# psweens/VAN-GAN

Measured on AMD Instinct MI355X. Metric: train Mvoxels/s (VanGan.train_step, 128^3 bf16), higher is better.
Workload: dtype bf16; 1 GPU; VanGan.train_step, 128x128x128 volumes, batch 1 per GPU (global 1), clDice on, disc noise+dropout on; parallelism=dp1

## Files before the change

include/vangan_hip.h:

```cpp
#ifndef VANGAN_HIP_H
#define VANGAN_HIP_H
#include <stdint.h>
#ifdef __cplusplus
extern "C" {
#endif

typedef void* vg_stream_t;

#define VG_OK 0
#define VG_EINVAL (-1)
#define VG_ELDS (-2)
#define VG_ELAUNCH (-3)

#define VG_ACT_NONE 0
#define VG_ACT_RELU 1
#define VG_ACT_LRELU 2

#define VG_PAD_ZERO 0
#define VG_PAD_REFLECT 1

#define VG_MAX_TAPS 64

#define VG_STRIPES 8

const char* vg_status_string(int code);
int vg_set_stamp_buffer(void* dev_u64);
int vg_version(void);
int vg_storage16(void);
int vg_abi_sizeof(int which);

struct vg_actnorm_bwd_desc_s;
typedef struct {
    const float* gamma; const float* beta;
    const float* mult;
    float* scale; float* shift;
    float* mean; float* rstd;
    int32_t c_off, c_tot;
} vg_fin_job;
typedef struct {
    uint32_t* ticket;
    float count;
    float eps;
    int32_t njobs;
    vg_fin_job job[2];
} vg_fin_desc;
typedef struct {
    const void* src0;
    const void* src1;
    int32_t c_src0, c_src1;
    int32_t src0_shift;
    int32_t src_f32;
    int32_t N, D, H, W;
    const float* in_scale;
    const float* in_shift;
    int32_t act;
    const void* noise;
    int32_t noise_pad;
    int32_t istr;
    int32_t pad_mode;
    int32_t ntaps;
    int8_t tap_d[VG_MAX_TAPS], tap_h[VG_MAX_TAPS], tap_w[VG_MAX_TAPS];
    int32_t OD, OH, OW;
    int32_t ostr, ooff_d, ooff_h, ooff_w;
    int32_t BD, BH, BW;
    int32_t Cout;
    const void* wpacked;
    int32_t CK;
    const float* bias;
    const void* res;
    const float* res_scale;
    const float* res_shift;
    int32_t tanh_out;
    void* out;
    int32_t out_f32;
    int32_t accumulate;
    float* out_sums;
    int32_t f32;
    int32_t nclass;
    int32_t cls_tap0[9];
    const void* cls_w[8];
    int32_t cls_ooff[8][3];
    int32_t cls_iters[8][3];
    int32_t wpack;
    int32_t wpack_wmin;
    const struct vg_actnorm_bwd_desc_s* bstat;
    void* scratch;
    int64_t scratch_bytes;
    int32_t wlayout;
    const vg_fin_desc* fin;
    int32_t res_c1;
    const void* wpacked_up;
} vg_conv_desc;
#define VG_SCRATCH_CTR_BYTES 16384

int vg_conv3d(const vg_conv_desc* d, vg_stream_t stream);

int vg_conv3d_lds_bytes(const vg_conv_desc* d);
int vg_conv3d_plan(const vg_conv_desc* d, int32_t* plan4);
int vg_conv3d_thin_np(const vg_conv_desc* d);
int vg_conv3d_variant(const vg_conv_desc* d, char* buf, int buflen);
int vg_set_tuning(const char* key, int value, int reset);

int vg_pack_up_weights(const float* w, int Cin, int Cout, int c_up, void* out, vg_stream_t stream);

int vg_pack_weights(const float* w, int T, int Cin, int Cout, const int32_t* tap_idx_dev, int ntaps,
                    int transpose, int CK, void* out, int out_f32, vg_stream_t stream);
typedef struct {
    const float* w; const int32_t* tap_idx; void* out;
    int32_t Cin, Cout, ntaps, transpose, CK, out_f32;
    int32_t blk0, nblk;
    int32_t bn;
    int32_t pad_;
} vg_pack_item;
int vg_pack_weights_multi(const vg_pack_item* items_dev, int n, int total_blocks, vg_stream_t stream);
int vg_conv3d_dma_bn(const vg_conv_desc* d);
int64_t vg_conv3d_scratch_bytes(const vg_conv_desc* d);
int vg_pack_weights_dma(const float* w, int T, int Cin, int Cout, const int32_t* tap_idx_dev, int ntaps, int transpose, int bn,
                        void* out, vg_stream_t stream);
int vg_packed_ktot(int ntaps, int C, int CK);
int vg_packed_rows(int N);

int vg_conv3d_wgrad(const vg_conv_desc* d, const void* dy, int dy_f32, const int32_t* tap_idx_host,
                    int T_total, float* dw, float* db, float* scratch, int64_t scratch_bytes, vg_stream_t stream);
int vg_conv3d_wgrad_variant(const vg_conv_desc* d, int dy_f32, const int32_t* tap_idx_host, int T_total,
                            int64_t scratch_bytes, char* buf, int buflen);

int vg_in_finalize(const float* sums0, int c0, float count0, const float* sums1, int c1, float count1,
                   const float* gamma, const float* beta, const float* mult, int N, float eps,
                   float* scale, float* shift, float* mean, float* rstd, vg_stream_t stream);

typedef struct vg_actnorm_bwd_desc_s {
    const void* g; int32_t g_padded;
    const void* x; int32_t x_f32;
    const void* x1; int32_t c_x0; int32_t x0_shift;
    int32_t N, D, H, W, C;
    const float* scale; const float* shift;
    const float* mult;
    int32_t act; int32_t norm;
    const float* gamma; const float* mean; const float* rstd;
    float* red;
    void* dx; int32_t dx_f32; int32_t accumulate;
    int32_t dx_cstride, dx_coff;
    int32_t f32;
    float* dgamma;
    float* dbeta;
    int32_t* ticket;
    int32_t alias_n0, alias_shift, pgrad_n, pad_;
} vg_actnorm_bwd_desc;
int vg_actnorm_bwd_stats(const vg_actnorm_bwd_desc* d, vg_stream_t stream);
int vg_actnorm_bwd_apply(const vg_actnorm_bwd_desc* d, vg_stream_t stream);
int vg_actnorm_bwd_apply2(const vg_actnorm_bwd_desc* d1, const vg_actnorm_bwd_desc* d2, vg_stream_t stream);
int vg_actnorm_bwd(const vg_actnorm_bwd_desc* d, vg_stream_t stream);
int vg_stem_short_fwd_workgroups(int N, int64_t S);
int vg_stem_short_fwd(const float* x, int N, int64_t S, int C, const float* w, const float* gamma, const float* beta, float eps, int round16,
                      float* scale, float* shift, double* part, int G, unsigned* ticket, vg_stream_t stream);
int vg_stem_short_bwd_workgroups(int N, int64_t S, int C);
int vg_stem_short_bwd(const void* g, int g_f32, const float* x, int N, int64_t S, int C, const float* w, const float* gamma, float eps,
                      int round16, float* dw, float* dgamma, float* dbeta, double* part, int G, unsigned* ticket, vg_stream_t stream);
int vg_in_param_grads(const float* red, int N, int C, float* dgamma, float* dbeta, vg_stream_t stream);

int vg_concat_bwd(const void* g, int N, int D, int H, int W, int Cu, int Cs, void* dlow, void* dskip,
                  int f32, int accumulate, vg_stream_t stream);

int vg_shortcut_dgrad_concat(const vg_conv_desc* d, void* dlow, void* dskip, int c_low, int accumulate, vg_stream_t stream);
int vg_shortcut_dgrad_concat_norm(const vg_conv_desc* d, const vg_actnorm_bwd_desc* b, void* dlow, void* dskip, int c_low,
                                  int accumulate, vg_stream_t stream);

int vg_affine_add(const void* a, const float* a_scale, const float* a_shift, int a_act, const void* b, const float* b_scale,
                  const float* b_shift, int N, int64_t S, int C, void* out, int f32, vg_stream_t stream);

int vg_bias_grad(const void* dy, int f32, int64_t rows, int C, float* db, vg_stream_t stream);

int vg_pack_cell_weights(const float* w, int C, void* out, vg_stream_t stream);
int vg_cells_fold(const void* cells, int N, int D, int H, int W, float* dx, vg_stream_t stream);

int vg_tanh_bwd(const float* dy, const float* y, float* dpre, int64_t n, vg_stream_t stream);

int vg_minmax(const float* x, int B, int64_t S, float* mm4, vg_stream_t stream);
int vg_minmax_apply(const float* x, const float* mm4, int B, int64_t S, float* y, vg_stream_t stream);
int vg_minmax_bwd(const float* x, const float* y, const float* gy, const float* mm4, int B, int64_t S,
                  float* tmp2, float* dx, vg_stream_t stream);
int vg_bce(const float* t, const float* p, int64_t n, float* acc, float gscale, float* gp, int accumulate,
           vg_stream_t stream);
int vg_mse(const float* a, const float* b, int64_t n, float* acc, float gscale, float* gb, int accumulate,
           vg_stream_t stream);
int vg_mse_const(const void* x, int x_f32, float target, int64_t n, float* acc, float gscale, float* gx,
                 int accumulate, vg_stream_t stream);
int vg_ssim_fwd(const float* t, const float* p, int B, int D, int H, int W, float* acc, float* part,
                vg_stream_t stream);
int vg_ssim_bwd(const float* t, const float* p, const float* part, int B, int D, int H, int W, float gscale,
                float* gp, int accumulate, vg_stream_t stream);

int vg_soft_skel_fwd(const float* img, int B, int D, int H, int W, int iters, float* imgs, float* skels, void* aux,
                     vg_stream_t stream);
int vg_soft_skel_bwd(const float* imgs, const float* skels, const float* gskel, int B, int D, int H, int W,
                     int iters, float* work, float* gimg, const void* aux, vg_stream_t stream);
int vg_cldice_coef(const float* sums7, float w, float alpha, float* coef6, vg_stream_t stream);
int vg_cldice_grads(const float* t, const float* skel_t, const float* coef6, int64_t n, float* gskel_p, float* gp,
                    int accumulate, vg_stream_t stream);
int vg_dot_sums(const float* a, const float* b, int64_t n, float* sums3, vg_stream_t stream);
int vg_axpby(const float* a, float alpha, const float* b, float beta, int64_t n, float* y, int accumulate,
             vg_stream_t stream);

int vg_dense_head_fwd(const float* x, const float* mask, const float* w, const float* b, int N, int n, float* z, vg_stream_t stream);
int vg_dense_head_bwd(const float* x, const float* mask, const float* w, const float* gz, int N, int n, float* dx, float* dw, float* db,
                      vg_stream_t stream);
int vg_wasserstein_terms(const float* z, int B, float inv, float* acc2, float* gz_d, float* gz_g, vg_stream_t stream);

int vg_overlap_add(const float* win, int kx, int ky, int kz, int px, int py, int pz, int x0, int y0, int z0,
                   int X, int Y, int Z, float* pred, float* cnt, vg_stream_t stream);
int vg_divide_crop(const float* pred, const float* cnt, int X, int Y, int Z, int sx, int sy, int sz, int ox, int oy,
                   int oz, float* out, vg_stream_t stream);

int vg_adam_clip(float* w, const float* g, float* m, float* v, const int64_t* seg_off_dev, int T,
                 int64_t total, float* norms, float lr_t, float beta1, float beta2, float eps,
                 float clipnorm, float grad_scale, vg_stream_t stream);

#define VG_SN_MAX_ITEMS 8
#define VG_SN_MAX_PROJ 4
#define VG_SN_MAX_COUT 512
#define VG_SN_SLAB 65536
#define VG_SN_STATE 8
#define VG_SN_STATE_CUM 4
typedef struct {
    float* w; float* u; float* state;
    int32_t K, Cout;
    int32_t blk0, nblk;
} vg_sn_item;
int vg_spectral_norm_blocks(int K, int Cout);
int64_t vg_spectral_norm_scratch_bytes(int total_blocks);
int vg_spectral_norm(const vg_sn_item* items_dev, int T, int total_blocks, int n_proj, float* scratch, int64_t scratch_bytes,
                     vg_stream_t stream);

int vg_attn_gate_fwd(const void* skip, const void* phi, const float* w_theta, const float* b_theta, const float* w_psi,
                     const float* b_psi, int N, int D, int H, int W, int Cs, int Ci, int f32, void* gated, float* h, float* sums,
                     vg_stream_t stream);
int vg_attn_gate_bwd(const void* dg, const void* skip, const float* h, const void* phi, const float* w_theta,
                     const float* b_theta, const float* w_psi, int N, int D, int H, int W, int Cs, int Ci, int f32, void* dskip,
                     int accumulate, void* dphi, float* dw_theta, float* db_theta, float* dw_psi, float* db_psi,
                     vg_stream_t stream);

int vg_randn_bf16_dev(void* out, int64_t n, const float* std_dev, uint64_t seed, const uint64_t* offset_dev, uint64_t offset_add,
                      vg_stream_t stream);
int vg_dropout_mask_dev(float* out, int64_t n, float rate, uint64_t seed, const uint64_t* offset_dev, uint64_t offset_add,
                        vg_stream_t stream);
int vg_adam_clip_dev(float* w, const float* g, float* m, float* v, const int64_t* seg_off_dev, int T, int64_t total, float* norms,
                     const float* lr_t_dev, float beta1, float beta2, float eps, float clipnorm, float grad_scale, vg_stream_t stream);

int vg_set_step_params(void* block, uint64_t offset, float std, float lr0, float lr1, float lr2, float lr3, vg_stream_t stream);

int vg_local_exchange(float* buf, float* scratch, int64_t n, int workgroups, int min_us, vg_stream_t stream);

int vg_randn_bf16(void* out, int64_t n, float std, uint64_t seed, uint64_t offset, vg_stream_t stream);
int vg_dropout_mask(float* out, int64_t n, float rate, uint64_t seed, uint64_t offset, vg_stream_t stream);

int vg_crop_augment(const float* vol, int X, int Y, int Z, int C, int x0, int y0, int z0, int px, int py, int pz,
                    int flip_lr, int flip_ud, int rot_k, float* out, vg_stream_t stream);
int vg_crop_max(const float* vol, int X, int Y, int Z, int C, int x0, int y0, int z0, int px, int py, int pz,
                float* out, vg_stream_t stream);

int vg_memset_zero(void* p, int64_t nbytes, vg_stream_t stream);
int vg_copy_bytes(void* dst, const void* src, int64_t nbytes, vg_stream_t stream);

int vg_f32_to_bf16(const float* x, void* y, int64_t n, vg_stream_t stream);
int vg_bf16_to_f32(const void* x, float* y, int64_t n, vg_stream_t stream);

#ifdef __cplusplus
}
#endif
#endif
```

van_gan_amd/_lib.py:

```python
from __future__ import annotations

import ctypes as C
import os

import torch

from . import build as _build

VG_MAX_TAPS = 64
SN_STATE, SN_STATE_CUM, SN_MAX_PROJ = 8, 4, 4
ACT_NONE, ACT_RELU, ACT_LRELU = 0, 1, 2
PAD_ZERO, PAD_REFLECT = 0, 1
SCRATCH_CTR_BYTES = 16384

c_void_p, c_int, c_float, c_i64, c_u64 = C.c_void_p, C.c_int32, C.c_float, C.c_int64, C.c_uint64


class ConvDesc(C.Structure):
    _fields_ = [
        ('src0', c_void_p), ('src1', c_void_p), ('c_src0', c_int), ('c_src1', c_int), ('src0_shift', c_int),
        ('src_f32', c_int), ('N', c_int), ('D', c_int), ('H', c_int), ('W', c_int),
        ('in_scale', c_void_p), ('in_shift', c_void_p), ('act', c_int), ('noise', c_void_p), ('noise_pad', c_int),
        ('istr', c_int), ('pad_mode', c_int), ('ntaps', c_int),
        ('tap_d', C.c_int8 * VG_MAX_TAPS), ('tap_h', C.c_int8 * VG_MAX_TAPS), ('tap_w', C.c_int8 * VG_MAX_TAPS),
        ('OD', c_int), ('OH', c_int), ('OW', c_int), ('ostr', c_int), ('ooff_d', c_int), ('ooff_h', c_int),
        ('ooff_w', c_int), ('BD', c_int), ('BH', c_int), ('BW', c_int), ('Cout', c_int),
        ('wpacked', c_void_p), ('CK', c_int), ('bias', c_void_p),
        ('res', c_void_p), ('res_scale', c_void_p), ('res_shift', c_void_p), ('tanh_out', c_int),
        ('out', c_void_p), ('out_f32', c_int), ('accumulate', c_int), ('out_sums', c_void_p), ('f32', c_int),
        ('nclass', c_int), ('cls_tap0', c_int * 9), ('cls_w', c_void_p * 8), ('cls_ooff', (c_int * 3) * 8),
        ('cls_iters', (c_int * 3) * 8), ('wpack', c_int), ('wpack_wmin', c_int), ('bstat', c_void_p),
        ('scratch', c_void_p), ('scratch_bytes', c_i64), ('wlayout', c_int), ('fin', c_void_p), ('res_c1', c_int), ('wpacked_up', c_void_p),
    ]


class FinJob(C.Structure):
    _fields_ = [('gamma', c_void_p), ('beta', c_void_p), ('mult', c_void_p), ('scale', c_void_p), ('shift', c_void_p),
                ('mean', c_void_p), ('rstd', c_void_p), ('c_off', c_int), ('c_tot', c_int)]


class FinDesc(C.Structure):
    _fields_ = [('ticket', c_void_p), ('count', c_float), ('eps', c_float), ('njobs', c_int), ('job', FinJob * 2)]


class PackItem(C.Structure):
    _fields_ = [('w', c_void_p), ('tap_idx', c_void_p), ('out', c_void_p), ('Cin', c_int), ('Cout', c_int), ('ntaps', c_int),
                ('transpose', c_int), ('CK', c_int), ('out_f32', c_int), ('blk0', c_int), ('nblk', c_int), ('bn', c_int), ('pad_', c_int)]


class SnItem(C.Structure):
    _fields_ = [('w', c_void_p), ('u', c_void_p), ('state', c_void_p), ('K', c_int), ('Cout', c_int), ('blk0', c_int), ('nblk', c_int)]


class ActNormBwdDesc(C.Structure):
    _fields_ = [
        ('g', c_void_p), ('g_padded', c_int), ('x', c_void_p), ('x_f32', c_int),
        ('x1', c_void_p), ('c_x0', c_int), ('x0_shift', c_int),
        ('N', c_int), ('D', c_int), ('H', c_int), ('W', c_int), ('C', c_int),
        ('scale', c_void_p), ('shift', c_void_p), ('mult', c_void_p), ('act', c_int), ('norm', c_int),
        ('gamma', c_void_p), ('mean', c_void_p), ('rstd', c_void_p), ('red', c_void_p),
        ('dx', c_void_p), ('dx_f32', c_int), ('accumulate', c_int), ('dx_cstride', c_int), ('dx_coff', c_int),
        ('f32', c_int), ('dgamma', c_void_p), ('dbeta', c_void_p), ('ticket', c_void_p),
        ('alias_n0', c_int), ('alias_shift', c_int), ('pgrad_n', c_int), ('pad_', c_int),
    ]


_SIGS = {
    'vg_version': ([], c_int),
    'vg_storage16': ([], c_int),
    'vg_abi_sizeof': ([c_int], c_int),
    'vg_set_stamp_buffer': ([c_void_p], c_int),
    'vg_conv3d': ([C.POINTER(ConvDesc), c_void_p], c_int),
    'vg_conv3d_lds_bytes': ([C.POINTER(ConvDesc)], c_int),
    'vg_conv3d_plan': ([C.POINTER(ConvDesc), C.POINTER(C.c_int32)], c_int),
    'vg_conv3d_variant': ([C.POINTER(ConvDesc), C.c_char_p, c_int], c_int),
    'vg_conv3d_thin_np': ([C.POINTER(ConvDesc)], c_int),
    'vg_set_tuning': ([C.c_char_p, c_int, c_int], c_int),
    'vg_conv3d_wgrad_variant': ([C.POINTER(ConvDesc), c_int, C.POINTER(c_int), c_int, c_i64, C.c_char_p, c_int], c_int),
    'vg_pack_weights': ([c_void_p, c_int, c_int, c_int, c_void_p, c_int, c_int, c_int, c_void_p, c_int, c_void_p], c_int),
    'vg_pack_weights_multi': ([c_void_p, c_int, c_int, c_void_p], c_int),
    'vg_crop_augment': ([c_void_p] + [c_int] * 13 + [c_void_p, c_void_p], c_int),
    'vg_crop_max': ([c_void_p] + [c_int] * 10 + [c_void_p, c_void_p], c_int),
    'vg_conv3d_dma_bn': ([C.POINTER(ConvDesc)], c_int),
    'vg_conv3d_scratch_bytes': ([C.POINTER(ConvDesc)], c_i64),
    'vg_pack_weights_dma': ([c_void_p, c_int, c_int, c_int, c_void_p, c_int, c_int, c_int, c_void_p, c_void_p], c_int),
    'vg_packed_ktot': ([c_int, c_int, c_int], c_int),
    'vg_packed_rows': ([c_int], c_int),
    'vg_conv3d_wgrad': ([C.POINTER(ConvDesc), c_void_p, c_int, C.POINTER(c_int), c_int, c_void_p, c_void_p, c_void_p, c_i64,
                         c_void_p], c_int),
    'vg_in_finalize': ([c_void_p, c_int, c_float, c_void_p, c_int, c_float, c_void_p, c_void_p, c_void_p, c_int,
                        c_float, c_void_p, c_void_p, c_void_p, c_void_p, c_void_p], c_int),
    'vg_actnorm_bwd_stats': ([C.POINTER(ActNormBwdDesc), c_void_p], c_int),
    'vg_actnorm_bwd_apply': ([C.POINTER(ActNormBwdDesc), c_void_p], c_int),
    'vg_actnorm_bwd_apply2': ([C.POINTER(ActNormBwdDesc), C.POINTER(ActNormBwdDesc), c_void_p], c_int),
    'vg_actnorm_bwd': ([C.POINTER(ActNormBwdDesc), c_void_p], c_int),
    'vg_stem_short_fwd_workgroups': ([c_int, c_i64], c_int),
    'vg_stem_short_fwd': ([c_void_p, c_int, c_i64, c_int, c_void_p, c_void_p, c_void_p, C.c_float, c_int, c_void_p, c_void_p, c_void_p, c_int, c_void_p,
                          c_void_p], c_int),
    'vg_stem_short_bwd_workgroups': ([c_int, c_i64, c_int], c_int),
    'vg_stem_short_bwd': ([c_void_p, c_int, c_void_p, c_int, c_i64, c_int, c_void_p, c_void_p, C.c_float, c_int, c_void_p, c_void_p, c_void_p,
                          c_void_p, c_int, c_void_p, c_void_p], c_int),
    'vg_in_param_grads': ([c_void_p, c_int, c_int, c_void_p, c_void_p, c_void_p], c_int),
    'vg_concat_bwd': ([c_void_p, c_int, c_int, c_int, c_int, c_int, c_int, c_void_p, c_void_p, c_int, c_int, c_void_p], c_int),
    'vg_shortcut_dgrad_concat': ([C.POINTER(ConvDesc), c_void_p, c_void_p, c_int, c_int, c_void_p], c_int),
    'vg_shortcut_dgrad_concat_norm': ([C.POINTER(ConvDesc), C.POINTER(ActNormBwdDesc), c_void_p, c_void_p, c_int, c_int, c_void_p], c_int),
    'vg_affine_add': ([c_void_p, c_void_p, c_void_p, c_int, c_void_p, c_void_p, c_void_p, c_int, c_i64, c_int, c_void_p, c_int, c_void_p], c_int),
    'vg_bias_grad': ([c_void_p, c_int, c_i64, c_int, c_void_p, c_void_p], c_int),
    'vg_pack_cell_weights': ([c_void_p, c_int, c_void_p, c_void_p], c_int),
    'vg_cells_fold': ([c_void_p, c_int, c_int, c_int, c_int, c_void_p, c_void_p], c_int),
    'vg_tanh_bwd': ([c_void_p, c_void_p, c_void_p, c_i64, c_void_p], c_int),
    'vg_minmax': ([c_void_p, c_int, c_i64, c_void_p, c_void_p], c_int),
    'vg_minmax_apply': ([c_void_p, c_void_p, c_int, c_i64, c_void_p, c_void_p], c_int),
    'vg_minmax_bwd': ([c_void_p, c_void_p, c_void_p, c_void_p, c_int, c_i64, c_void_p, c_void_p, c_void_p], c_int),
    'vg_bce': ([c_void_p, c_void_p, c_i64, c_void_p, c_float, c_void_p, c_int, c_void_p], c_int),
    'vg_mse': ([c_void_p, c_void_p, c_i64, c_void_p, c_float, c_void_p, c_int, c_void_p], c_int),
    'vg_mse_const': ([c_void_p, c_int, c_float, c_i64, c_void_p, c_float, c_void_p, c_int, c_void_p], c_int),
    'vg_ssim_fwd': ([c_void_p, c_void_p, c_int, c_int, c_int, c_int, c_void_p, c_void_p, c_void_p], c_int),
    'vg_ssim_bwd': ([c_void_p, c_void_p, c_void_p, c_int, c_int, c_int, c_int, c_float, c_void_p, c_int, c_void_p], c_int),
    'vg_soft_skel_fwd': ([c_void_p, c_int, c_int, c_int, c_int, c_int, c_void_p, c_void_p, c_void_p, c_void_p], c_int),
    'vg_soft_skel_bwd': ([c_void_p, c_void_p, c_void_p, c_int, c_int, c_int, c_int, c_int, c_void_p, c_void_p, c_void_p, c_void_p], c_int),
    'vg_cldice_coef': ([c_void_p, c_float, c_float, c_void_p, c_void_p], c_int),
    'vg_cldice_grads': ([c_void_p, c_void_p, c_void_p, c_i64, c_void_p, c_void_p, c_int, c_void_p], c_int),
    'vg_dense_head_fwd': ([c_void_p, c_void_p, c_void_p, c_void_p, c_int, c_int, c_void_p, c_void_p], c_int),
    'vg_dense_head_bwd': ([c_void_p, c_void_p, c_void_p, c_void_p, c_int, c_int, c_void_p, c_void_p, c_void_p, c_void_p], c_int),
    'vg_wasserstein_terms': ([c_void_p, c_int, c_float, c_void_p, c_void_p, c_void_p, c_void_p], c_int),
    'vg_dot_sums': ([c_void_p, c_void_p, c_i64, c_void_p, c_void_p], c_int),
    'vg_overlap_add': ([c_void_p] + [c_int] * 12 + [c_void_p, c_void_p, c_void_p], c_int),
    'vg_divide_crop': ([c_void_p, c_void_p] + [c_int] * 9 + [c_void_p, c_void_p], c_int),
    'vg_axpby': ([c_void_p, c_float, c_void_p, c_float, c_i64, c_void_p, c_int, c_void_p], c_int),
    'vg_adam_clip': ([c_void_p, c_void_p, c_void_p, c_void_p, c_void_p, c_int, c_i64, c_void_p, c_float, c_float,
                      c_float, c_float, c_float, c_float, c_void_p], c_int),
    'vg_spectral_norm_blocks': ([c_int, c_int], c_int),
    'vg_spectral_norm_scratch_bytes': ([c_int], c_i64),
    'vg_spectral_norm': ([c_void_p, c_int, c_int, c_int, c_void_p, c_i64, c_void_p], c_int),
    'vg_attn_gate_fwd': ([c_void_p] * 6 + [c_int] * 7 + [c_void_p] * 4, c_int),
    'vg_attn_gate_bwd': ([c_void_p] * 7 + [c_int] * 7 + [c_void_p, c_int] + [c_void_p] * 6, c_int),
    'vg_local_exchange': ([c_void_p, c_void_p, c_i64, c_int, c_int, c_void_p], c_int),
    'vg_randn_bf16': ([c_void_p, c_i64, c_float, c_u64, c_u64, c_void_p], c_int),
    'vg_dropout_mask': ([c_void_p, c_i64, c_float, c_u64, c_u64, c_void_p], c_int),
    'vg_randn_bf16_dev': ([c_void_p, c_i64, c_void_p, c_u64, c_void_p, c_u64, c_void_p], c_int),
    'vg_dropout_mask_dev': ([c_void_p, c_i64, c_float, c_u64, c_void_p, c_u64, c_void_p], c_int),
    'vg_adam_clip_dev': ([c_void_p, c_void_p, c_void_p, c_void_p, c_void_p, c_int, c_i64, c_void_p, c_void_p, c_float,
                          c_float, c_float, c_float, c_float, c_void_p], c_int),
    'vg_set_step_params': ([c_void_p, c_u64, c_float, c_float, c_float, c_float, c_float, c_void_p], c_int),
    'vg_pack_up_weights': ([c_void_p, c_int, c_int, c_int, c_void_p, c_void_p], c_int),
    'vg_memset_zero': ([c_void_p, c_i64, c_void_p], c_int),
    'vg_copy_bytes': ([c_void_p, c_void_p, c_i64, c_void_p], c_int),
    'vg_f32_to_bf16': ([c_void_p, c_void_p, c_i64, c_void_p], c_int),
    'vg_bf16_to_f32': ([c_void_p, c_void_p, c_i64, c_void_p], c_int),
}

EXPORTS = sorted(list(_SIGS.keys()) + ['vg_status_string'])


def _load(path=None, storage16=0):
    path = _build.LIB if path is None else path
    if not os.path.exists(path) or (_build.needs_build() and os.environ.get('VG_NO_REBUILD') != '1'):
        _build.build()
    lib = C.CDLL(path)
    for name, (args, ret) in _SIGS.items():
        fn = getattr(lib, name)
        fn.argtypes = args
        fn.restype = ret
    lib.vg_status_string.argtypes = [c_int]
    lib.vg_status_string.restype = C.c_char_p
    for which, mirror in ((0, ConvDesc), (1, ActNormBwdDesc), (2, PackItem), (3, FinDesc), (4, SnItem)):
        got = lib.vg_abi_sizeof(which)
        if got != C.sizeof(mirror):
            raise ImportError('libvangan_hip.so ABI mismatch: sizeof(%s) is %d in the library, %d in van_gan_amd/_lib.py '
                              '(stale build? remove %s and rebuild)' % (mirror.__name__, got, C.sizeof(mirror), path))
    if lib.vg_storage16() != storage16:
        raise ImportError('%s stores %s in its 16-bit buffers, expected %s' % (path, ('bf16', 'fp16')[lib.vg_storage16()], ('bf16', 'fp16')[storage16]))
    return lib


lib = _load()
_lib_h = None


def lib_fp16():
    global _lib_h
    if _lib_h is None:
        _lib_h = _load(_build.LIB_H, 1)
    return _lib_h


class VgError(RuntimeError):
    pass


def check(rc: int, what: str = '') -> int:
    if rc < 0:
        raise VgError('%s failed: %s (%d)' % (what or 'libvangan_hip call', lib.vg_status_string(rc).decode(), rc))
    return rc
```

van_gan_amd/csrc/vg_pointwise.hip:

```cpp
#include "vg_common.h"
#include "vg_c1k3.h"
#include <stdlib.h>

namespace {

struct PW {
    const void* x; int x_f32;
    const float* scale; const float* shift; int act;
    const void* w; int kc_pad, CK;
    const float* bias;
    void* out; int out_f32, accumulate, tanh_out;
    float* sums;
    const void* dy; int dy_f32;
    float* dw; float* db;
    int N, C; int64_t S;
    VgFin fin;
};

__device__ __forceinline__ float pw_slope(int act) { return act == VG_ACT_RELU ? 0.f : (act == VG_ACT_LRELU ? VG_LRELU : 1.f); }
__device__ __forceinline__ float ld_single(const void* p, int f32, int64_t i) {
    return f32 ? ld_global((const float*)p + i) : ld_global((const bf16_t*)p + i);
}

template <typename T, int G>
// ... 27 lines not shown
                float x[8]; raw_unpack(r[k][g], x);
#pragma unroll
                for (int j = 0; j < 8; ++j) {
                    float y = x[j] * sc[g * 8 + j] + sf[g * 8 + j];
                    y = fmaxf(y, y * slope);
                    a += rnd<T>(y) * wv[g * 8 + j];
                }
            }
            const size_t o = (size_t)n * p.S + v + k * stride;
            if (p.tanh_out && !p.accumulate) a = tanhf(a);
            if (p.out_f32) { float* q = (float*)p.out + o; a = p.accumulate ? *q + a : a; *q = a; }
            else { bf16_t* q = (bf16_t*)p.out + o; const bf16_t h = f2bf(p.accumulate ? bf2f(*q) + a : a); *q = h; a = bf2f(h); }
            s1 += a; s2 += a * a;
        }
    }
    if (p.sums) {
        __shared__ float red[8];
#pragma unroll
        for (int o = 32; o > 0; o >>= 1) { s1 += __shfl_xor(s1, o); s2 += __shfl_xor(s2, o); }
        if ((threadIdx.x & 63) == 0) { red[(threadIdx.x >> 6) * 2] = s1; red[(threadIdx.x >> 6) * 2 + 1] = s2; }
        __syncthreads();
        if (threadIdx.x < 2) {
            const int stripe = blockIdx.x & (VG_STRIPES - 1);
            atomicAdd(&p.sums[((size_t)stripe * gridDim.y + n) * 2 + threadIdx.x],
                      red[threadIdx.x] + red[2 + threadIdx.x] + red[4 + threadIdx.x] + red[6 + threadIdx.x]);
        }
    }
}

template <typename T>
__global__ __launch_bounds__(256) void pw_1toc_kernel(const PW p) {
    __shared__ float part[16 * 256];
    const int n = blockIdx.y, tid = threadIdx.x;
    const int gpc = p.C >> 3, vpb = 256 / gpc;
    const int cg = tid % gpc, vl = tid / gpc;
    const bool live = tid < gpc * vpb;
    float wv[8], bv[8], s1[8], s2[8];
#pragma unroll
    for (int j = 0; j < 8; ++j) {
        wv[j] = live ? ld1<T>((const T*)p.w + (size_t)(cg * 8 + j) * p.kc_pad) : 0.f;
        bv[j] = (live && p.bias) ? p.bias[cg * 8 + j] : 0.f;
        s1[j] = 0.f; s2[j] = 0.f;
    }
    const float sc = p.scale ? p.scale[n] : 1.f, sf = p.scale ? p.shift[n] : 0.f, slope = pw_slope(p.act);
    const int64_t xoff = (int64_t)n * p.S;
    T* ob = (T*)p.out + (size_t)n * p.S * p.C + cg * 8;
    const int64_t stride = (int64_t)gridDim.x * vpb;
    if (live)
    for (int64_t v = (int64_t)blockIdx.x * vpb + vl; v < p.S; v += 4 * stride) {
        float xs[4]; Raw8<T> old[4];
#pragma unroll
        for (int k = 0; k < 4; ++k) {
            const int64_t vv = v + k * stride < p.S ? v + k * stride : v;
            xs[k] = ld_single(p.x, p.x_f32, xoff + vv);
            if (p.accumulate) raw_load(old[k], ob + vv * p.C);
        }
#pragma unroll
        for (int k = 0; k < 4; ++k) {
            if (v + k * stride >= p.S) continue;
            float y = xs[k] * sc + sf;
            y = rnd<T>(fmaxf(y, y * slope));
            float o[8];
#pragma unroll
            for (int j = 0; j < 8; ++j) o[j] = y * wv[j] + bv[j];
            if (p.accumulate) {
                float q[8]; raw_unpack(old[k], q);
#pragma unroll
                for (int j = 0; j < 8; ++j) o[j] += q[j];
            }
            store8<T>(ob + (v + k * stride) * p.C, o);
#pragma unroll
            for (int j = 0; j < 8; ++j) { const float r = rnd<T>(o[j]); s1[j] += r; s2[j] += r * r; }
        }
    }
    if (!p.sums) return;
#pragma unroll
    for (int j = 0; j < 8; ++j) { part[(2 * j) * 256 + tid] = live ? s1[j] : 0.f; part[(2 * j + 1) * 256 + tid] = live ? s2[j] : 0.f; }
    __syncthreads();
    const int stripe = blockIdx.x & (VG_STRIPES - 1);
    float* dst = p.sums + ((size_t)stripe * gridDim.y + n) * p.C * 2;
    for (int o = tid; o < p.C * 2; o += 256) {
        const int ch = o >> 1, mom = o & 1, g8 = ch >> 3, j = ch & 7;
        const float* src = part + (2 * j + mom) * 256 + g8;
        float a = 0.f;
        for (int t = 0; t < vpb; ++t) a += src[t * gpc];
        atomicAdd(&dst[o], a);
    }
    if (p.fin.ticket) vg_fin_tail(p.fin, p.sums, gridDim.y, p.C, gridDim.x * gridDim.y, (int*)part);
}

template <typename T, int GI>
__global__ __launch_bounds__(256) void pw_ctoc_kernel(const PW p, int Cin, int Ktot) {
    const int n = blockIdx.y, tid = threadIdx.x;
    const int gpc = p.C >> 3, vpb = 256 / gpc;
    const int cg = tid % gpc, vl = tid / gpc;
    if (tid >= gpc * vpb) return;
    float wv[GI * 8][8], bv[8];
#pragma unroll
    for (int k = 0; k < GI * 8; ++k)
#pragma unroll
        for (int j = 0; j < 8; ++j)
            wv[k][j] = ld1<T>((const T*)p.w + (size_t)(cg * 8 + j) * Ktot + (k / p.CK) * p.kc_pad + (k % p.CK));
#pragma unroll
    for (int j = 0; j < 8; ++j) bv[j] = p.bias ? p.bias[cg * 8 + j] : 0.f;
    const T* xb = (const T*)p.x + (size_t)n * p.S * Cin;
    T* ob = (T*)p.out + (size_t)n * p.S * p.C + cg * 8;
    const int64_t stride = (int64_t)gridDim.x * vpb;
    for (int64_t v = (int64_t)blockIdx.x * vpb + vl; v < p.S; v += 2 * stride) {
        Raw8<T> xr[2][GI], old[2];
#pragma unroll
        for (int k = 0; k < 2; ++k) {
            const int64_t vv = v + k * stride < p.S ? v + k * stride : v;
#pragma unroll
            for (int g = 0; g < GI; ++g) raw_load(xr[k][g], xb + vv * Cin + g * 8);
            if (p.accumulate) raw_load(old[k], ob + vv * p.C);
        }
#pragma unroll
        for (int k = 0; k < 2; ++k) {
            if (v + k * stride >= p.S) continue;
            float o[8];
#pragma unroll
            for (int j = 0; j < 8; ++j) o[j] = bv[j];
#pragma unroll
            for (int g = 0; g < GI; ++g) {
                float x[8]; raw_unpack(xr[k][g], x);
#pragma unroll
                for (int e = 0; e < 8; ++e)
#pragma unroll
                    for (int j = 0; j < 8; ++j) o[j] += x[e] * wv[g * 8 + e][j];
            }
            if (p.accumulate) {
                float q[8]; raw_unpack(old[k], q);
#pragma unroll
                for (int j = 0; j < 8; ++j) o[j] += q[j];
            }
            store8<T>(ob + (v + k * stride) * p.C, o);
        }
    }
}

struct PWG {
    const bf16_t* x0; const bf16_t* x1; int c0, c1, Cin, sh;
    const bf16_t* w; int Ktot, CK, kc_pad;
    const float* bias; bf16_t* out; float* sums;
    int N, ID, IH, IW, OD, OH, OW, istr;
    int BD, BH, BW, ostr, od0, oh0, ow0;
    int Cout; int SO;
    unsigned long long* stamps;
    bf16_t* dlow; bf16_t* dskip; int sc0, sacc;
    const bf16_t* ng; const bf16_t* nx0; const bf16_t* nx1;
    const float* n_scale; const float* n_shift; const float* n_mean; const float* n_rstd; const float* n_gamma; const float* n_mult;
    VgFin fin;
    const float* n_red; float* n_dgamma; float* n_dbeta; int n_act;
};
}
extern unsigned long long* g_vg_stamps;
namespace {
typedef __attribute__((ext_vector_type(2))) float pw_f32x2;
typedef __attribute__((ext_vector_type(2))) unsigned pw_u32x2;
typedef __attribute__((ext_vector_type(4))) unsigned pw_u32x4;

__device__ __forceinline__ void vg_reflect_fold8(const bf16_t* gp, int C, int D, int H, int W, int dk, int hk, int wk, float* g) {
    const int PH = H + 2, PW_ = W + 2;
    const int md = dk == 1 ? 0 : (dk == D - 2 ? D + 1 : -1), mh = hk == 1 ? 0 : (hk == H - 2 ? H + 1 : -1), mw = wk == 1 ? 0 : (wk == W - 2 ? W + 1 : -1);
    Raw8<bf16_t> rr[7];
    bool val[7];
#pragma unroll
    for (int t = 1; t < 8; ++t) {
        const int qd = (t & 4) ? md : dk + 1, qh = (t & 2) ? mh : hk + 1, qw = (t & 1) ? mw : wk + 1;
        val[t - 1] = (qd | qh | qw) >= 0;
        raw_load(rr[t - 1], gp + (val[t - 1] ? ((size_t)(qd * PH + qh) * PW_ + qw) * C : ((size_t)((dk + 1) * PH + hk + 1) * PW_ + wk + 1) * C));
    }
#pragma unroll
    for (int t = 0; t < 7; ++t) {
        float r[8]; raw_unpack(rr[t], r);
#pragma unroll
        for (int j = 0; j < 8; ++j) g[j] += val[t] ? r[j] : 0.f;
    }
}

template <int KS, int NB, bool GEO, bool ACC, bool STATS, int SPLIT = 0>
__global__ __launch_bounds__(256) void pw_gemm_kernel(const PWG p) {
    static_assert(!SPLIT || (ACC && !GEO && !STATS), "SPLIT: accumulating, same-grid launches");
    constexpr int MS = (KS * NB <= 2) ? 4 : 2;
    __shared__ float stat[NB * 32];
    const int tid = threadIdx.x, lane = tid & 63, wave = tid >> 6, r = lane & 15, kg = lane >> 4;
    const int n = blockIdx.y;
    if (p.stamps && lane == 0) p.stamps[((size_t)blockIdx.x * 4 + wave) * 8] = __builtin_amdgcn_s_memrealtime();
    float* ntab = nullptr;
    if constexpr (SPLIT == 2) {
        __shared__ float ntab_s[5 * NB * 16];
        ntab = ntab_s;
        constexpr int C = NB * 16;
        if (tid < C && tid < p.Cout) {
            const int nc = n * p.Cout + tid;
            const size_t total = (size_t)p.N * p.Cout * 2;
            float r0 = 0.f, r1 = 0.f;
#pragma unroll
            for (int t = 0; t < VG_STRIPES; ++t) { r0 += p.n_red[t * total + (size_t)nc * 2]; r1 += p.n_red[t * total + (size_t)nc * 2 + 1]; }
            if (p.n_dgamma && blockIdx.x == 0) { atomicAdd(&p.n_dbeta[tid], r0); atomicAdd(&p.n_dgamma[tid], r1); }
            const float cnt = (float)p.SO, rs = p.n_rstd[nc], mu = p.n_mean[nc], gr = p.n_gamma[tid] * rs;
            const float k1 = gr * r0 / cnt, k2 = gr * r1 / cnt, cc = k2 * rs;
            ntab_s[tid] = p.n_scale ? p.n_scale[nc] : 1.f;
            ntab_s[C + tid] = p.n_scale ? p.n_shift[nc] : 0.f;
            ntab_s[2 * C + tid] = gr * (p.n_mult ? p.n_mult[nc] : 1.f);
            ntab_s[3 * C + tid] = k1 - cc * mu;
            ntab_s[4 * C + tid] = cc;
        }
        __syncthreads();
    }
    bf16x8 wA[NB][KS];
    pw_f32x2 e_b[NB][2];
#pragma unroll
    for (int nb = 0; nb < NB; ++nb) {
        const int co = nb * 16 + r;
#pragma unroll
        for (int ks = 0; ks < KS; ++ks) {
            const int c = ks * 32 + kg * 8;
            wA[nb][ks] = (bf16x8){0, 0, 0, 0, 0, 0, 0, 0};
            if (co < p.Cout && c < p.Cin) wA[nb][ks] = *(const bf16x8*)(p.w + (size_t)co * p.Ktot + (c / p.CK) * p.kc_pad + (c % p.CK));
        }
#pragma unroll
        for (int i = 0; i < 4; ++i) {
            const int cb = nb * 16 + kg * 4 + i;
            e_b[nb][i >> 1][i & 1] = (p.bias && cb < p.Cout) ? p.bias[cb] : 0.f;
        }
    }
    if (p.stamps) { asm volatile("s_waitcnt vmcnt(0)" ::: "memory"); if (lane == 0) p.stamps[((size_t)blockIdx.x * 4 + wave) * 8 + 1] = __builtin_amdgcn_s_memrealtime(); }
    float s1[NB][4], s2[NB][4];
#pragma unroll
    for (int nb = 0; nb < NB; ++nb)
#pragma unroll
        for (int i = 0; i < 4; ++i) { s1[nb][i] = 0.f; s2[nb][i] = 0.f; }
    if (STATS) { if (tid < NB * 32) stat[tid] = 0.f; __syncthreads(); }
    const int OHW = p.OH * p.OW;
    const int ID2 = p.ID >> p.sh, IH2 = p.IH >> p.sh, IW2 = p.IW >> p.sh;
    const int nwt = (p.SO + MS * 16 - 1) / (MS * 16);
    const int jodd = kg & 1, chof = (kg & ~1) * 4;
    auto split_store = [&](int wt, int jp, int nb, float* o, bool ok, size_t vox) {
        if (nb * 16 < p.sc0) {
#pragma unroll
            for (int i = 0; i < 8; ++i) { o[i] += __shfl_xor(o[i], 1); o[i] += __shfl_xor(o[i], 2); o[i] += __shfl_xor(o[i], 4); }
            if (ok && (r & 7) == 0) {
                const size_t cidx = (size_t)n * (p.SO >> 3) + (size_t)wt * (MS * 2) + (jp + jodd) * 2 + (r >> 3);
                bf16_t* dst = p.dlow + cidx * p.sc0 + nb * 16 + chof;
                if (p.sacc & 1) { float old[8]; load8<bf16_t>(dst, old); for (int i = 0; i < 8; ++i) o[i] += old[i]; }
                store8<bf16_t>(dst, o);
            }
        } else if (ok) {
            bf16_t* dst = p.dskip + vox * (p.Cout - p.sc0) + (nb * 16 - p.sc0) + chof;
            if (p.sacc & 2) { float old[8]; load8<bf16_t>(dst, old); for (int i = 0; i < 8; ++i) o[i] += old[i]; }
            store8<bf16_t>(dst, o);
        }
    };
    for (int wt = blockIdx.x * 4 + wave; wt < nwt; wt += gridDim.x * 4) {
        bf16x8 xb[MS][KS];
        bool vok[MS], oks[MS / 2];
        size_t i0s[MS], i1s[MS], ovs[MS / 2];
        size_t ovf[MS / 2];
        int fdhw[MS / 2];
#pragma unroll
        for (int jp = 0; jp < MS; jp += 2) {
            size_t ovp[2];
#pragma unroll
            for (int e = 0; e < 2; ++e) {
                const int i = jp + e;
                const int v = wt * (MS * 16) + i * 16 + r;
                vok[i] = v < p.SO;
                const int vc = vok[i] ? v : p.SO - 1;
                if (GEO) {
                    const int od = vc / OHW, rem = vc - od * OHW, oh = rem / p.OW, ow = rem - oh * p.OW;
                    const int id = od * p.istr, ih = oh * p.istr, iw = ow * p.istr;
                    i0s[i] = (((size_t)n * ID2 + (id >> p.sh)) * IH2 + (ih >> p.sh)) * IW2 + (iw >> p.sh);
                    i1s[i] = (((size_t)n * p.ID + id) * p.IH + ih) * p.IW + iw;
                    ovp[e] = (((size_t)n * p.BD + od * p.ostr + p.od0) * p.BH + oh * p.ostr + p.oh0) * p.BW + ow * p.ostr + p.ow0;
                } else if (SPLIT) {
                    const int cb = vc >> 3, j = vc & 7;
                    const int CW = p.OW >> 1, CHW = (p.OH >> 1) * CW;
                    const int cd = cb / CHW, rem = cb - cd * CHW, ch = rem / CW, cw = rem - ch * CW;
                    const int fd = 2 * cd + (j >> 2), fh = 2 * ch + ((j >> 1) & 1), fw = 2 * cw + (j & 1);
                    const int vf = (fd * p.OH + fh) * p.OW + fw;
                    i0s[i] = i1s[i] = ovp[e] = (size_t)n * p.SO + vf;
                    if (e == jodd) fdhw[jp >> 1] = fd | (fh << 10) | (fw << 20);
                } else {
                    i0s[i] = i1s[i] = ovp[e] = (size_t)n * p.SO + vc;
                }
            }
            ovf[jp >> 1] = jodd ? ovp[1] : ovp[0];
            ovs[jp >> 1] = (jodd ? ovp[1] : ovp[0]) * p.Cout + chof;
            oks[jp >> 1] = jodd ? vok[jp + 1] : vok[jp];
        }
        Raw8<bf16_t> oldv[ACC ? MS / 2 : 1][ACC ? NB : 1];
        if (ACC && SPLIT != 2) {
#pragma unroll
            for (int jh = 0; jh < MS / 2; ++jh)
#pragma unroll
                for (int nb = 0; nb < NB; ++nb) raw_load(oldv[jh][nb], p.out + ovs[jh] + (nb * 16 < p.Cout ? nb * 16 : 0));
            if (p.stamps) { asm volatile("s_waitcnt vmcnt(0)" ::: "memory"); if (lane == 0) p.stamps[((size_t)blockIdx.x * 4 + wave) * 8 + 3] = __builtin_amdgcn_s_memrealtime(); }
        }
#pragma unroll
        for (int i = 0; i < MS; ++i)
#pragma unroll
            for (int ks = 0; ks < KS; ++ks) {
                const int c = ks * 32 + kg * 8;
                const bool cok = c < p.Cin;
                const int ce = cok ? c : c % p.Cin;
                const bf16_t* q = ce < p.c0 ? p.x0 + i0s[i] * p.c0 + ce : p.x1 + i1s[i] * p.c1 + (ce - p.c0);
                Raw8<bf16_t> t;
                raw_load(t, q);
                raw_mask(t, cok);
                xb[i][ks] = t.v;
            }
        if (p.stamps) { asm volatile("s_waitcnt vmcnt(0)" ::: "memory"); if (lane == 0) p.stamps[((size_t)blockIdx.x * 4 + wave) * 8 + 2] = __builtin_amdgcn_s_memrealtime(); }
        if constexpr (SPLIT == 2) {
            const int PH = p.OH + 2, PW_ = p.OW + 2;
            size_t gi[MS / 2], li[MS / 2], si[MS / 2];
            bool bord[MS / 2];
#pragma unroll
            for (int jh = 0; jh < MS / 2; ++jh) {
                const int fd = fdhw[jh] & 1023, fh = (fdhw[jh] >> 10) & 1023, fw = fdhw[jh] >> 20;
                gi[jh] = ((((size_t)n * (p.OD + 2) + fd + 1) * PH + fh + 1) * PW_ + fw + 1) * p.Cout + chof;
                li[jh] = ((((size_t)n * (p.OD >> 1) + (fd >> 1)) * (p.OH >> 1) + (fh >> 1)) * (p.OW >> 1) + (fw >> 1)) * p.sc0 + chof;
                si[jh] = ovf[jh] * (p.Cout - p.sc0) + chof;
                bord[jh] = fd == 1 || fd == p.OD - 2 || fh == 1 || fh == p.OH - 2 || fw == 1 || fw == p.OW - 2;
            }
            constexpr int C = NB * 16;
            const float slope = pw_slope(p.n_act);
            Raw8<bf16_t> gq[NB][MS / 2], xq[NB][MS / 2];
#pragma unroll
            for (int nb = 0; nb < NB; ++nb)
#pragma unroll
                for (int jh = 0; jh < MS / 2; ++jh) {
                    raw_load(gq[nb][jh], p.ng + gi[jh] + nb * 16);
                    raw_load(xq[nb][jh], nb * 16 < p.sc0 ? p.nx0 + li[jh] + nb * 16 : p.nx1 + si[jh] + (nb * 16 - p.sc0));
                }
#pragma unroll
            for (int nb = 0; nb < NB; ++nb) {
                f32x4 a[MS];
#pragma unroll
                for (int i = 0; i < MS; ++i) {
                    a[i] = (f32x4){0.f, 0.f, 0.f, 0.f};
#pragma unroll
                    for (int ks = 0; ks < KS; ++ks) a[i] = VG_MFMA16(wA[nb][ks], xb[i][ks], a[i]);
                }
                const float* tb = ntab + nb * 16 + chof;
#pragma unroll
                for (int jp = 0; jp < MS; jp += 2) {
                    float o[8];
#pragma unroll
                    for (int i = 0; i < 4; ++i) {
                        const pw_u32x2 x = __builtin_amdgcn_permlane16_swap(__float_as_uint(a[jp][i]), __float_as_uint(a[jp + 1][i]), false, false);
                        o[i] = __uint_as_float(x[0]); o[4 + i] = __uint_as_float(x[1]);
                    }
                    float q[8], xv[8];
                    raw_unpack(gq[nb][jp >> 1], q); raw_unpack(xq[nb][jp >> 1], xv);
                    if (bord[jp >> 1]) {
                        const int fd = fdhw[jp >> 1] & 1023, fh = (fdhw[jp >> 1] >> 10) & 1023, fw = fdhw[jp >> 1] >> 20;
                        vg_reflect_fold8(p.ng + (size_t)n * (p.OD + 2) * PH * PW_ * p.Cout + nb * 16 + chof, p.Cout, p.OD, p.OH, p.OW, fd, fh, fw, q);
                    }
#pragma unroll
                    for (int i = 0; i < 8; ++i) {
                        const float pre = xv[i] * tb[i] + tb[C + i];
                        const float m = (pre > 0.f || p.n_act == VG_ACT_NONE) ? 1.f : slope;
                        o[i] += tb[2 * C + i] * m * q[i] - tb[3 * C + i] - tb[4 * C + i] * xv[i];
                    }
                    split_store(wt, jp, nb, o, oks[jp >> 1], ovf[jp >> 1]);
                }
                __builtin_amdgcn_sched_barrier(0);
            }
            continue;
        }
        f32x4 acc[MS][NB];
#pragma unroll
        for (int i = 0; i < MS; ++i)
#pragma unroll
            for (int nb = 0; nb < NB; ++nb) {
                acc[i][nb] = (f32x4){0.f, 0.f, 0.f, 0.f};
#pragma unroll
                for (int ks = 0; ks < KS; ++ks) acc[i][nb] = VG_MFMA16(wA[nb][ks], xb[i][ks], acc[i][nb]);
            }
#pragma unroll
        for (int jp = 0; jp < MS; jp += 2) {
            const bool ok = oks[jp >> 1];
            const size_t ob = ovs[jp >> 1];
#pragma unroll
            for (int nb = 0; nb < NB; ++nb) {
                if (nb * 16 >= p.Cout) continue;
                bf16_t* optr = p.out + ob + nb * 16;
                pw_u32x4 outv;
                if (ACC) {
                    float o[8];
#pragma unroll
                    for (int i = 0; i < 4; ++i) {
                        const pw_u32x2 x = __builtin_amdgcn_permlane16_swap(__float_as_uint(acc[jp][nb][i] + e_b[nb][i >> 1][i & 1]),
                                                                            __float_as_uint(acc[jp + 1][nb][i] + e_b[nb][i >> 1][i & 1]), false, false);
                        o[i] = __uint_as_float(x[0]); o[4 + i] = __uint_as_float(x[1]);
                    }
                    float q[8]; raw_unpack(oldv[ACC ? jp >> 1 : 0][ACC ? nb : 0], q);
                    if (SPLIT) {
#pragma unroll
                        for (int i = 0; i < 8; ++i) o[i] += q[i];
                        split_store(wt, jp, nb, o, ok, ovf[jp >> 1]);
                        continue;
                    }
                    bf16x8 pk;
#pragma unroll
                    for (int i = 0; i < 8; ++i) pk[i] = (short)f2bf(o[i] + q[i]);
                    outv = __builtin_bit_cast(pw_u32x4, pk);
                } else {
                    bf16x4 pk[2];
#pragma unroll
                    for (int e = 0; e < 2; ++e) {
                        pw_f32x2 v0 = {acc[jp + e][nb][0], acc[jp + e][nb][1]}, v1 = {acc[jp + e][nb][2], acc[jp + e][nb][3]};
                        v0 += e_b[nb][0]; v1 += e_b[nb][1];
                        pk[e] = (bf16x4){(short)f2bf(v0[0]), (short)f2bf(v0[1]), (short)f2bf(v1[0]), (short)f2bf(v1[1])};
                        if (STATS) {
                            const bool okv = vok[jp + e];
#pragma unroll
                            for (int i = 0; i < 4; ++i) {
                                const float qv = okv ? bf2f((bf16_t)pk[e][i]) : 0.f;
                                s1[nb][i] += qv; s2[nb][i] += qv * qv;
                            }
                        }
                    }
                    const pw_u32x2 wa = __builtin_bit_cast(pw_u32x2, pk[0]), wb = __builtin_bit_cast(pw_u32x2, pk[1]);
                    const pw_u32x2 x0 = __builtin_amdgcn_permlane16_swap(wa[0], wb[0], false, false);
                    const pw_u32x2 x1 = __builtin_amdgcn_permlane16_swap(wa[1], wb[1], false, false);
                    outv = (pw_u32x4){x0[0], x1[0], x0[1], x1[1]};
                }
                if (ok) *(pw_u32x4*)optr = outv;
            }
        }
    }
    if (p.stamps && lane == 0) { asm volatile("s_waitcnt vmcnt(0)" ::: "memory"); p.stamps[((size_t)blockIdx.x * 4 + wave) * 8 + 7] = __builtin_amdgcn_s_memrealtime(); }
    if (STATS && p.sums) {
#pragma unroll
        for (int nb = 0; nb < NB; ++nb)
#pragma unroll
            for (int i = 0; i < 4; ++i) {
                float a = s1[nb][i], b = s2[nb][i];
#pragma unroll
                for (int o = 1; o < 16; o <<= 1) { a += __shfl_xor(a, o); b += __shfl_xor(b, o); }
                if (r == 0) { atomicAdd(&stat[(nb * 16 + 4 * kg + i) * 2], a); atomicAdd(&stat[(nb * 16 + 4 * kg + i) * 2 + 1], b); }
            }
        __syncthreads();
        if (tid < NB * 32) {
            const int co = tid >> 1;
            const int stripe = blockIdx.x & (VG_STRIPES - 1);
            if (co < p.Cout) atomicAdd(&p.sums[(((size_t)stripe * gridDim.y + n) * p.Cout + co) * 2 + (tid & 1)], stat[tid]);
        }
        if (p.fin.ticket) vg_fin_tail(p.fin, p.sums, gridDim.y, p.Cout, gridDim.x * gridDim.y, (int*)stat);
    }
}

struct PWW {
    const bf16_t* x0; const bf16_t* x1; int c0, c1, Cin, sh;
    const bf16_t* dy; int Cout;
    int N, ID, IH, IW, OD, OH, OW, istr, SO;
    int gin, roles, rp, vpb;
    float* dw; float* db; float* part; int dw_elems;
};

__global__ __launch_bounds__(256) void pw_wgrad_cc_kernel(const PWW p) {
    __shared__ float red[4 * 64 * 16];
    const int tid = threadIdx.x, n = blockIdx.y;
    const int role = tid & (p.rp - 1), vl = tid / p.rp;
    const bool live = role < p.roles;
    const int rl = live ? role : 0;
    const int cg = rl % p.gin, cob = rl / p.gin, c = cg * 8;
    const bool from0 = c < p.c0;
    const float bmask = cg == 0 ? 1.f : 0.f;
    pw_f32x2 acc[8][8], bs[8];
#pragma unroll
    for (int i = 0; i < 8; ++i) {
        bs[i] = (pw_f32x2){0.f, 0.f};
#pragma unroll
        for (int j = 0; j < 8; ++j) acc[i][j] = (pw_f32x2){0.f, 0.f};
    }
    const int ID2 = p.ID >> p.sh, IH2 = p.IH >> p.sh, IW2 = p.IW >> p.sh;
    const int step = gridDim.x * p.vpb;
    int v = blockIdx.x * p.vpb + vl;
    const int OHW = p.OH * p.OW;
    int od = v / OHW, oh = (v - od * OHW) / p.OW, ow = v - od * OHW - oh * p.OW;
    const int sd = step / OHW, sh_ = (step - sd * OHW) / p.OW, sw = step - sd * OHW - sh_ * p.OW;
    const bf16_t* xb = from0 ? p.x0 + c : p.x1 + (c - p.c0);
    const int cs = from0 ? p.c0 : p.c1, shx = from0 ? p.sh : 0;
    const int XD = from0 ? ID2 : p.ID, XH = from0 ? IH2 : p.IH, XW = from0 ? IW2 : p.IW;
    const bf16_t* yb = p.dy + (size_t)n * p.SO * p.Cout + cob * 16;
// ... 224 lines not shown
        atomicAdd(&dst[o], a);
    }
    if (p.fin.ticket) vg_fin_tail(p.fin, p.sums, gridDim.y, p.C, gridDim.x * gridDim.y, (int*)part);
}

template <typename T, typename S>
__global__ __launch_bounds__(256) void c1k3_wgrad_kernel(C1K3 p) {
    __shared__ float part[20 * 256];
    const int n = blockIdx.y, tid = threadIdx.x;
    const int gpc = p.C >> 3, roles = 3 * gpc, qpb = 256 / roles;
    const int role = tid % roles, cg = role % gpc, a = role / gpc, ql = tid / roles;
    const bool live = tid < roles * qpb;
    if (p.scale) { p.sc = p.scale[n]; p.sf = p.shift[n]; }
    float acc[80];
#pragma unroll
    for (int i = 0; i < 80; ++i) acc[i] = 0.f;
    const int64_t nq = (int64_t)p.D * p.H * p.W4;
    if (live)
    for (int64_t q = (int64_t)blockIdx.x * qpb + ql; q < nq; q += (int64_t)gridDim.x * qpb) {
        const int wq = (int)(q % p.W4); const int64_t r = q / p.W4;
        const int h = (int)(r % p.H), d = (int)(r / p.H), w0 = wq * 4;
        float xv[1][3][6];
        c1_window<T, S, 1>(p, n, d, h, w0, a, xv);
        const T* yb = (const T*)p.dy + (((size_t)n * p.D + d) * p.H + h) * p.W * p.C + cg * 8;
        Raw8<T> yr[4];
#pragma unroll
        for (int v = 0; v < 4; ++v) raw_load(yr[v], yb + (size_t)min(w0 + v, p.W - 1) * p.C);
#pragma unroll
        for (int v = 0; v < 4; ++v) {
            float g[8]; raw_unpack(yr[v], g);
            const bool okv = w0 + v < p.W;
#pragma unroll
            for (int c = 0; c < 8; ++c) g[c] = okv ? g[c] : 0.f;
#pragma unroll
            for (int b = 0; b < 3; ++b)
#pragma unroll
                for (int j = 0; j < 3; ++j) {
                    const float x = xv[0][b][v + j];
#pragma unroll
                    for (int c = 0; c < 8; ++c) acc[(b * 3 + j) * 8 + c] += x * g[c];
                }
            if (a == 0) {
#pragma unroll
                for (int c = 0; c < 8; ++c) acc[72 + c] += g[c];
            }
        }
    }
#pragma unroll
    for (int chunk = 0; chunk < 4; ++chunk) {
        __syncthreads();
#pragma unroll
        for (int i = 0; i < 20; ++i) part[i * 256 + tid] = live ? acc[chunk * 20 + i] : 0.f;
        __syncthreads();
        for (int o = tid; o < roles * 20; o += 256) {
            const int i = o / roles, ro = o - i * roles;
            const float* src = part + i * 256 + ro;
            float sacc = 0.f;
            for (int t = 0; t < qpb; ++t) sacc += src[t * roles];
            const int val = chunk * 20 + i, rcg = ro % gpc, ra = ro / gpc;
            if (val < 72) {
                const int b = val / 24, j = (val / 8) % 3, c = val & 7;
                atomicAdd(&p.dw[(size_t)(((ra * 3 + b) * 3) + j) * p.C + rcg * 8 + c], sacc);
            } else if (ra == 0 && p.db) atomicAdd(&p.db[rcg * 8 + (val - 72)], sacc);
        }
    }
}

bool c1k3_fill(const vg_conv_desc* d, C1K3& p) {
    if (d->c_src0 != 1 || d->src1 || d->c_src1 || d->wpack != 3 || d->ntaps != 9 || d->istr != 1 || d->noise || d->nclass > 1) return false;
    if (d->Cout < 8 || d->Cout > 32 || (d->Cout % 8)) return false;
    if (d->OD != d->D || d->OH != d->H || d->OW != d->W) return false;
    for (int t = 0; t < 9; ++t)
        if (d->tap_d[t] != d->tap_d[0] + t / 3 || d->tap_h[t] != d->tap_h[0] + t % 3 || d->tap_w[t] != 0) return false;
    p.x = d->src0; p.x_f32 = d->src_f32; p.sc = 1.f; p.sf = 0.f; p.scale = d->in_scale; p.shift = d->in_shift; p.act = d->act;
    p.pad_mode = d->pad_mode; p.D = d->D; p.H = d->H; p.W = d->W; p.C = d->Cout; p.W4 = (d->W + 3) / 4;
    p.td0 = d->tap_d[0]; p.th0 = d->tap_h[0]; p.tw0 = d->wpack_wmin;
    p.CK = d->CK; p.Ktot = ((9 * d->CK + 31) / 32) * 32;
    return true;
}

bool pw_enabled() { return vg_tune("PW", 1) != 0; }
bool pw_shape_ok(const vg_conv_desc* d) {
    if (!pw_enabled() || d->ntaps != 1 || d->tap_d[0] || d->tap_h[0] || d->tap_w[0]) return false;
    if (d->istr != 1 || d->src1 || d->c_src1 || d->src0_shift || d->noise || d->wpack || d->nclass > 1) return false;
    if (d->OD != d->D || d->OH != d->H || d->OW != d->W) return false;
    return true;
}
int pw_blocks(int64_t work_items, int N) {
    int64_t b = (work_items + 255) / 256;
    const int64_t cap = 2047 / (N > 0 ? N : 1);
    if (b > cap) b = cap;
    return b < 1 ? 1 : (int)b;
}

template <bool GEO, bool ACC, bool STATS>
bool pwg_launch(int KS, int NB, dim3 grid, hipStream_t s, const PWG& p) {
#define PWG_CASE(ks, nb) if (KS == ks && NB == nb) { hipLaunchKernelGGL((pw_gemm_kernel<ks, nb, GEO, ACC, STATS>), grid, dim3(256), 0, s, p); return true; }
    PWG_CASE(1, 1) PWG_CASE(1, 2) PWG_CASE(1, 3) PWG_CASE(1, 4) PWG_CASE(1, 6) PWG_CASE(2, 1) PWG_CASE(2, 2) PWG_CASE(3, 2)
    PWG_CASE(4, 4) PWG_CASE(6, 4) PWG_CASE(2, 8)
#undef PWG_CASE
    return false;
}
template <int SPLIT>
bool pwg_launch_split(int KS, int NB, dim3 grid, hipStream_t s, const PWG& p) {
#define PWG_CASE(ks, nb) if (KS == ks && NB == nb) { hipLaunchKernelGGL((pw_gemm_kernel<ks, nb, false, true, false, SPLIT>), grid, dim3(256), 0, s, p); return true; }
    PWG_CASE(1, 3) PWG_CASE(1, 6) PWG_CASE(2, 6)
#undef PWG_CASE
    return false;
}
bool pwg_case_ok(int KS, int NB) {
    static const int tab[][2] = {{1, 1}, {1, 2}, {1, 3}, {1, 4}, {1, 6}, {2, 1}, {2, 2}, {3, 2}, {4, 4}, {6, 4}, {2, 8}};
    for (auto& t : tab) if (t[0] == KS && t[1] == NB) return true;
    return false;
}
int pw_gemm_conv(const vg_conv_desc* d, hipStream_t s) {
    if (!pw_enabled() || !vg_tune("PW_GEMM", 1)) return 1;
    if (d->ntaps != 1 || d->tap_d[0] || d->tap_h[0] || d->tap_w[0] || d->noise || d->wpack || d->nclass > 1) return 1;
    if (d->f32 || d->src_f32 || d->out_f32 || d->in_scale || d->act != VG_ACT_NONE || d->res || d->tanh_out) return 1;
    const int Cin = d->c_src0 + d->c_src1;
    if (Cin < 8 || (Cin % 8) || (d->c_src1 && (d->c_src0 % 8)) || d->Cout < 16 || (d->Cout % 16) || (d->CK % 8)) return 1;
    if (d->c_src1 && !d->src1) return 1;
    if (d->src0_shift && ((d->D | d->H | d->W) & 1)) return 1;
    if (d->istr < 1 || d->ostr < 1 || (d->OD - 1) * d->istr >= d->D || (d->OH - 1) * d->istr >= d->H || (d->OW - 1) * d->istr >= d->W) return 1;
    if (d->accumulate && d->out_sums) return 1;
    const int64_t SO = (int64_t)d->OD * d->OH * d->OW;
    if (SO < 1 || SO > (1 << 30)) return 1;
    const int KS = (Cin + 31) / 32, NB = d->Cout / 16;
    if (!pwg_case_ok(KS, NB)) return 1;
    const bool geo = d->src0_shift || d->istr != 1 || d->ostr != 1 || d->ooff_d || d->ooff_h || d->ooff_w || d->BD != d->OD || d->BH != d->OH
                     || d->BW != d->OW || d->OD != d->D || d->OH != d->H || d->OW != d->W;
    PWG p = {};
    p.x0 = (const bf16_t*)d->src0; p.x1 = (const bf16_t*)(d->c_src1 ? d->src1 : d->src0); p.c0 = d->c_src0; p.c1 = d->c_src1 ? d->c_src1 : 1;
    p.Cin = Cin; p.sh = d->src0_shift ? 1 : 0;
    p.w = (const bf16_t*)d->wpacked; p.CK = d->CK; p.kc_pad = ((d->CK + 31) / 32) * 32; p.Ktot = ((Cin + d->CK - 1) / d->CK) * p.kc_pad;
    p.bias = d->bias; p.out = (bf16_t*)d->out; p.sums = d->out_sums;
    p.N = d->N; p.ID = d->D; p.IH = d->H; p.IW = d->W; p.OD = d->OD; p.OH = d->OH; p.OW = d->OW; p.istr = d->istr;
    p.BD = d->BD; p.BH = d->BH; p.BW = d->BW; p.ostr = d->ostr; p.od0 = d->ooff_d; p.oh0 = d->ooff_h; p.ow0 = d->ooff_w;
    p.Cout = d->Cout; p.SO = (int)SO; p.stamps = g_vg_stamps;
    p.fin = vg_fin_of(d);
    const int MS = (KS * NB <= 2) ? 4 : 2;
    const int64_t nwt = (SO + MS * 16 - 1) / (MS * 16);
    int64_t b = (nwt + 3) / 4;
    const int capt = vg_tune("PW_GEMM_CAP", 2047);
    const int64_t cap = (capt / d->N) > 0 ? (capt / d->N) : 1;
    if (b > cap) b = cap;
    const dim3 grid((int)b, d->N);
    if (vg_dry("pw_gemm<%d,%d,g%d,a%d>", KS, NB, (geo || !d->accumulate) ? 1 : 0, d->accumulate ? 1 : 0)) return VG_OK;
    bool ok;
    if (!d->accumulate) { ok = pwg_launch<true, false, true>(KS, NB, grid, s, p); if (ok && p.sums && p.fin.ticket) vg_fin_done = true; }
    else ok = geo ? pwg_launch<true, true, false>(KS, NB, grid, s, p) : pwg_launch<false, true, false>(KS, NB, grid, s, p);
    return ok ? vg_check_launch() : 1;
}

int pw_gemm_split(const vg_conv_desc* d, const vg_actnorm_bwd_desc* nb_, void* dlow, void* dskip, int c_low, int acc, hipStream_t s) {
    if (!pw_enabled() || !vg_tune("PW_GEMM", 1) || !vg_tune("PW_SPLIT", 1)) return 1;
    if (d->ntaps != 1 || d->tap_d[0] || d->tap_h[0] || d->tap_w[0] || d->noise || d->wpack || d->nclass > 1) return 1;
    if (d->f32 || d->src_f32 || d->out_f32 || d->in_scale || d->act != VG_ACT_NONE || d->res || d->tanh_out || d->out_sums || d->bias) return 1;
    const int Cin = d->c_src0;
    if (d->c_src1 || d->src0_shift || Cin < 8 || (Cin % 8) || d->Cout < 32 || (d->Cout % 16) || (d->CK % 8) || (!d->accumulate && !nb_)) return 1;
    if (nb_) {
        if (!nb_->norm || !nb_->g_padded || nb_->f32 || nb_->x_f32 || !nb_->g || !nb_->x || !nb_->x1 || !nb_->x0_shift || nb_->c_x0 != c_low) return 1;
        if (nb_->C != d->Cout || nb_->N != d->N || nb_->D != d->D || nb_->H != d->H || nb_->W != d->W || !nb_->gamma || !nb_->mean || !nb_->rstd || !nb_->red) return 1;
        if (d->D < 4 || d->H < 4 || d->W < 4 || d->D > 1023 || d->H > 1023 || d->W > 1023) return 1;
    }
    if (c_low < 16 || (c_low % 16) || c_low >= d->Cout) return 1;
    if (d->istr != 1 || d->ostr != 1 || d->ooff_d || d->ooff_h || d->ooff_w || d->BD != d->OD || d->BH != d->OH || d->BW != d->OW
        || d->OD != d->D || d->OH != d->H || d->OW != d->W || ((d->D | d->H | d->W) & 1)) return 1;
    const int64_t SO = (int64_t)d->OD * d->OH * d->OW;
    if (SO < 8 || SO > (1 << 30)) return 1;
    const int KS = (Cin + 31) / 32, NB = d->Cout / 16;
    if (!((KS == 1 && (NB == 3 || NB == 6)) || (KS == 2 && NB == 6))) return 1;
    PWG p = {};
    p.x0 = (const bf16_t*)d->src0; p.x1 = p.x0; p.c0 = Cin; p.c1 = 1; p.Cin = Cin; p.sh = 0;
    p.w = (const bf16_t*)d->wpacked; p.CK = d->CK; p.kc_pad = ((d->CK + 31) / 32) * 32; p.Ktot = ((Cin + d->CK - 1) / d->CK) * p.kc_pad;
    p.bias = nullptr; p.out = (bf16_t*)d->out; p.sums = nullptr;
    p.N = d->N; p.ID = d->D; p.IH = d->H; p.IW = d->W; p.OD = d->OD; p.OH = d->OH; p.OW = d->OW; p.istr = 1;
    p.BD = d->BD; p.BH = d->BH; p.BW = d->BW; p.ostr = 1;
    p.Cout = d->Cout; p.SO = (int)SO; p.stamps = g_vg_stamps;
    p.dlow = (bf16_t*)dlow; p.dskip = (bf16_t*)dskip; p.sc0 = c_low; p.sacc = acc;
    if (nb_) {
        p.ng = (const bf16_t*)nb_->g; p.nx0 = (const bf16_t*)nb_->x; p.nx1 = (const bf16_t*)nb_->x1;
        p.n_scale = nb_->scale; p.n_shift = nb_->shift; p.n_mean = nb_->mean; p.n_rstd = nb_->rstd; p.n_gamma = nb_->gamma; p.n_mult = nb_->mult;
        p.n_red = nb_->red; p.n_dgamma = (nb_->dgamma && nb_->dbeta) ? nb_->dgamma : nullptr; p.n_dbeta = nb_->dbeta; p.n_act = nb_->act;
    }
    const int MS = (KS * NB <= 2) ? 4 : 2;
    const int64_t nwt = (SO + MS * 16 - 1) / (MS * 16);
    int64_t b = (nwt + 3) / 4;
    const int capt = vg_tune("PW_GEMM_CAP", 2047);
    const int64_t cap = (capt / d->N) > 0 ? (capt / d->N) : 1;
    if (b > cap) b = cap;
    if (vg_dry("pw_gemm_split<%d,%d,n%d>", KS, NB, nb_ ? 1 : 0)) return VG_OK;
    const bool ok = nb_ ? pwg_launch_split<2>(KS, NB, dim3((int)b, d->N), s, p) : pwg_launch_split<1>(KS, NB, dim3((int)b, d->N), s, p);
    return ok ? vg_check_launch() : 1;
}

int pw_wgrad_cc(const vg_conv_desc* d, const void* dy, int dy_f32, int T_total, float* dw, float* db, float* scratch,
                int64_t scratch_bytes, hipStream_t s) {
    if (!pw_enabled() || !vg_tune("PW_WGRAD_CC", 1)) return 1;
    if (T_total != 1 || d->ntaps != 1 || d->tap_d[0] || d->tap_h[0] || d->tap_w[0] || d->noise || d->wpack || d->nclass > 1) return 1;
    if (d->f32 || d->src_f32 || dy_f32 || d->in_scale || d->act != VG_ACT_NONE) return 1;
    const int Cin = d->c_src0 + d->c_src1;
    if (Cin < 8 || (Cin % 8) || (d->c_src1 && (d->c_src0 % 8)) || d->Cout < 16 || (d->Cout % 16)) return 1;
    if (d->c_src1 && !d->src1) return 1;
    if (d->src0_shift && ((d->D | d->H | d->W) & 1)) return 1;
    if (d->istr < 1 || (d->OD - 1) * d->istr >= d->D || (d->OH - 1) * d->istr >= d->H || (d->OW - 1) * d->istr >= d->W) return 1;
    const int64_t SO = (int64_t)d->OD * d->OH * d->OW;
    if (SO < 1 || SO > (1 << 30)) return 1;
    PWW p = {};
    p.gin = Cin / 8; p.roles = p.gin * (d->Cout / 16);
    if (p.roles > vg_tune("PW_WGRAD_ROLES", 16)) return 1;
    p.rp = pow2_ceil(p.roles); p.vpb = 256 / p.rp;
    p.x0 = (const bf16_t*)d->src0; p.x1 = (const bf16_t*)(d->c_src1 ? d->src1 : d->src0); p.c0 = d->c_src0; p.c1 = d->c_src1 ? d->c_src1 : 1;
    p.Cin = Cin; p.sh = d->src0_shift ? 1 : 0; p.dy = (const bf16_t*)dy; p.Cout = d->Cout;
    p.N = d->N; p.ID = d->D; p.IH = d->H; p.IW = d->W; p.OD = d->OD; p.OH = d->OH; p.OW = d->OW; p.istr = d->istr; p.SO = (int)SO;
    p.dw = dw; p.db = db; p.dw_elems = Cin * d->Cout;
    int64_t b = (SO + (int64_t)p.vpb * 8 - 1) / ((int64_t)p.vpb * 8);
    const int capt = vg_tune("PW_WGRAD_CAP", 511);
    const int64_t cap = (capt / d->N) > 0 ? (capt / d->N) : 1;
    if (b > cap) b = cap;
    if (b < 1) b = 1;
    const int nslab = (int)b * d->N;
    p.part = (nslab > 4 && scratch && (int64_t)nslab * p.dw_elems * 4 <= scratch_bytes) ? scratch : nullptr;
    if (vg_dry("pw_wgrad_cc<r%d>|part%d", p.roles, p.part ? 1 : 0)) return VG_OK;
    hipLaunchKernelGGL(pw_wgrad_cc_kernel, dim3((int)b, d->N), dim3(256), 0, s, p);
    if (p.part) vg_launch_reduce_partials(p.part, nslab, p.dw_elems, dw, s);
    return vg_check_launch();
}

}

extern "C" int vg_shortcut_dgrad_concat(const vg_conv_desc* d, void* dlow, void* dskip, int c_low, int accumulate, vg_stream_t stream) {
    vg_begin();
    if (!d || !d->src0 || !d->out || !d->wpacked || !dlow || !dskip) return VG_EINVAL;
    return pw_gemm_split(d, nullptr, dlow, dskip, c_low, accumulate, (hipStream_t)stream);
}
extern "C" int vg_shortcut_dgrad_concat_norm(const vg_conv_desc* d, const vg_actnorm_bwd_desc* b, void* dlow, void* dskip, int c_low,
                                             int accumulate, vg_stream_t stream) {
    vg_begin();
    if (!d || !b || !d->src0 || !d->wpacked || !dlow || !dskip) return VG_EINVAL;
    if (!vg_tune("PW_SPLIT_NORM", 1)) return 1;
    return pw_gemm_split(d, b, dlow, dskip, c_low, accumulate, (hipStream_t)stream);
}

int vg_pointwise_conv(const vg_conv_desc* d, hipStream_t s) {
    if (pw_enabled() && !d->res && !d->tanh_out && !d->accumulate && d->ostr == 1 && !d->ooff_d && !d->ooff_h && !d->ooff_w
        && d->BD == d->OD && d->BH == d->OH && d->BW == d->OW && !(d->out_f32 && !d->f32)) {
        { const int mrc = c1m_fwd(d, s); if (mrc <= 0) return mrc; }
        C1K3 c;
        if (c1k3_fill(d, c)) {
            c.w = d->wpacked; c.bias = d->bias; c.out = d->out; c.sums = d->out_sums;
            c.fin = vg_fin_of(d);
            const int qpb = 256 / (c.C >> 3);
            int64_t b = ((int64_t)c.D * c.H * c.W4 + qpb - 1) / qpb;
            const int64_t cap = (2047 / d->N) > 0 ? (2047 / d->N) : 1;
            if (b > cap) b = cap;
            const dim3 grid((int)b, d->N);
            if (vg_dry("c1k3_fwd<%s,%s>", d->f32 ? "f32" : "bf16", d->src_f32 ? "f32" : "bf16")) return VG_OK;
            if (d->f32) {
                if (d->src_f32) hipLaunchKernelGGL((c1k3_fwd_kernel<float, float>), grid, dim3(256), 0, s, c);
                else hipLaunchKernelGGL((c1k3_fwd_kernel<float, bf16_t>), grid, dim3(256), 0, s, c);
            } else {
                if (d->src_f32) hipLaunchKernelGGL((c1k3_fwd_kernel<bf16_t, float>), grid, dim3(256), 0, s, c);
                else hipLaunchKernelGGL((c1k3_fwd_kernel<bf16_t, bf16_t>), grid, dim3(256), 0, s, c);
            }
            if (c.sums && c.fin.ticket) vg_fin_done = true;
            return vg_check_launch();
        }
    }
    { const int grc = pw_gemm_conv(d, s); if (grc <= 0) return grc; }
    if (!pw_shape_ok(d) || d->res) return 1;
    if (d->ostr != 1 || d->ooff_d || d->ooff_h || d->ooff_w || d->BD != d->OD || d->BH != d->OH || d->BW != d->OW) return 1;
    if (d->tanh_out && d->accumulate) return 1;
    const int Cin = d->c_src0;
    PW p = {};
    p.x = d->src0; p.x_f32 = d->src_f32; p.scale = d->in_scale; p.shift = d->in_shift; p.act = d->act;
    p.w = d->wpacked; p.CK = d->CK; p.kc_pad = ((d->CK + 31) / 32) * 32;
    p.bias = d->bias; p.out = d->out; p.out_f32 = (d->out_f32 || d->f32) ? 1 : 0; p.accumulate = d->accumulate; p.tanh_out = d->tanh_out;
    p.sums = d->out_sums; p.N = d->N; p.S = (int64_t)d->D * d->H * d->W;
    if (d->Cout == 1 && Cin >= 8 && Cin <= 32 && (Cin % 8) == 0) {
        p.C = Cin;
        const dim3 grid(pw_blocks((p.S + 1) / 2, d->N), d->N);
        if (vg_dry("pw_cto1<%s,%d>", d->f32 ? "f32" : "bf16", Cin / 8 > 4 ? 4 : Cin / 8)) return VG_OK;
#define PW_CTO1(T)                                                                                                      \
        switch (Cin / 8) {                                                                                              \
            case 1: hipLaunchKernelGGL((pw_cto1_kernel<T, 1>), grid, dim3(256), 0, s, p); break;                        \
            case 2: hipLaunchKernelGGL((pw_cto1_kernel<T, 2>), grid, dim3(256), 0, s, p); break;                        \
            case 3: hipLaunchKernelGGL((pw_cto1_kernel<T, 3>), grid, dim3(256), 0, s, p); break;                        \
            default: hipLaunchKernelGGL((pw_cto1_kernel<T, 4>), grid, dim3(256), 0, s, p); break;                       \
        }
        if (d->f32) { PW_CTO1(float) } else { PW_CTO1(bf16_t) }
#undef PW_CTO1
        return vg_check_launch();
    }
    if (Cin == 1 && d->Cout >= 8 && d->Cout <= 256 && (d->Cout % 8) == 0 && !d->tanh_out && !(d->out_f32 && !d->f32)) {
        p.C = d->Cout;
        p.kc_pad = ((d->CK + 31) / 32) * 32;
        const int vpb = 256 / (p.C >> 3);
        const dim3 grid(pw_blocks((p.S + 3) / 4 * (256 / vpb), d->N), d->N);
        if (vg_dry("pw_1toc<%s>", d->f32 ? "f32" : "bf16")) return VG_OK;
        p.fin = vg_fin_of(d);
        if (d->f32) hipLaunchKernelGGL((pw_1toc_kernel<float>), grid, dim3(256), 0, s, p);
        else hipLaunchKernelGGL((pw_1toc_kernel<bf16_t>), grid, dim3(256), 0, s, p);
        if (p.sums && p.fin.ticket) vg_fin_done = true;
        return vg_check_launch();
    }
    if ((Cin == 8 || Cin == 16) && d->Cout >= 16 && d->Cout <= 128 && (d->Cout % 8) == 0 && !d->in_scale && d->act == VG_ACT_NONE
        && !d->tanh_out && !d->out_sums && !d->src_f32 && !(d->out_f32 && !d->f32)) {
        p.C = d->Cout;
        const int nchunks = (Cin + d->CK - 1) / d->CK;
        const int Ktot = nchunks * p.kc_pad;
        const int vpb = 256 / (p.C >> 3);
        const dim3 grid(pw_blocks((p.S + 1) / 2 * (256 / vpb), d->N), d->N);
        if (vg_dry("pw_ctoc<%s,%d>", d->f32 ? "f32" : "bf16", Cin / 8)) return VG_OK;
        if (d->f32) {
            if (Cin == 8) hipLaunchKernelGGL((pw_ctoc_kernel<float, 1>), grid, dim3(256), 0, s, p, Cin, Ktot);
            else hipLaunchKernelGGL((pw_ctoc_kernel<float, 2>), grid, dim3(256), 0, s, p, Cin, Ktot);
        } else {
            if (Cin == 8) hipLaunchKernelGGL((pw_ctoc_kernel<bf16_t, 1>), grid, dim3(256), 0, s, p, Cin, Ktot);
            else hipLaunchKernelGGL((pw_ctoc_kernel<bf16_t, 2>), grid, dim3(256), 0, s, p, Cin, Ktot);
        }
        return vg_check_launch();
    }
    return 1;
}

int vg_pointwise_wgrad(const vg_conv_desc* d, const void* dy, int dy_f32, int T_total, float* dw, float* db, float* scratch,
                       int64_t scratch_bytes, hipStream_t s) {
    if (pw_enabled()) { const int mrc = c1m_wgrad(d, dy, dy_f32, T_total, dw, db, scratch, scratch_bytes, s); if (mrc <= 0) return mrc; }
    if (pw_enabled() && T_total == 9 && !(dy_f32 && !d->f32)) {
        C1K3 c;
        if (c1k3_fill(d, c)) {
            c.dy = dy; c.dw = dw; c.db = db;
            const int qpb = 256 / (3 * (c.C >> 3));
            int64_t b = ((int64_t)c.D * c.H * c.W4 + (int64_t)qpb * 8 - 1) / ((int64_t)qpb * 8);
            const int64_t cap = (767 / d->N) > 0 ? (767 / d->N) : 1;
            if (b > cap) b = cap;
            if (b < 1) b = 1;
            const dim3 grid((int)b, d->N);
            if (vg_dry("c1k3_wgrad<%s,%s>", d->f32 ? "f32" : "bf16", d->src_f32 ? "f32" : "bf16")) return VG_OK;
            if (d->f32) {
                if (d->src_f32) hipLaunchKernelGGL((c1k3_wgrad_kernel<float, float>), grid, dim3(256), 0, s, c);
                else hipLaunchKernelGGL((c1k3_wgrad_kernel<float, bf16_t>), grid, dim3(256), 0, s, c);
            } else {
                if (d->src_f32) hipLaunchKernelGGL((c1k3_wgrad_kernel<bf16_t, float>), grid, dim3(256), 0, s, c);
                else hipLaunchKernelGGL((c1k3_wgrad_kernel<bf16_t, bf16_t>), grid, dim3(256), 0, s, c);
            }
            return vg_check_launch();
        }
    }
    { const int wrc = pw_wgrad_cc(d, dy, dy_f32, T_total, dw, db, scratch, scratch_bytes, s); if (wrc <= 0) return wrc; }
    if (!pw_shape_ok(d) || T_total != 1) return 1;
    const int Cin = d->c_src0;
    PW p = {};
    p.x = d->src0; p.x_f32 = d->src_f32; p.scale = d->in_scale; p.shift = d->in_shift; p.act = d->act;
    p.dy = dy; p.dy_f32 = dy_f32; p.dw = dw; p.db = db; p.N = d->N; p.S = (int64_t)d->D * d->H * d->W;
    const bool c_to_1 = d->Cout == 1 && Cin >= 8 && Cin <= 256 && (Cin % 8) == 0;
    const bool one_to_c = Cin == 1 && d->Cout >= 8 && d->Cout <= 256 && (d->Cout % 8) == 0 && !(dy_f32 && !d->f32);
    if (!c_to_1 && !one_to_c) return 1;
    p.C = c_to_1 ? Cin : d->Cout;
    const int vpb = 256 / (p.C >> 3);
    int64_t b = (p.S + (int64_t)vpb * 16 - 1) / ((int64_t)vpb * 16);
    const int64_t cap = (511 / d->N) > 0 ? (511 / d->N) : 1;
    if (b > cap) b = cap;
    if (b < 1) b = 1;
    const dim3 grid((int)b, d->N);
    if (vg_dry("pw_wgrad<%s,%s>", d->f32 ? "f32" : "bf16", c_to_1 ? "cto1" : "1toc")) return VG_OK;
    if (c_to_1) {
        if (d->f32) hipLaunchKernelGGL((pw_wgrad_kernel<float, true>), grid, dim3(256), 0, s, p);
        else hipLaunchKernelGGL((pw_wgrad_kernel<bf16_t, true>), grid, dim3(256), 0, s, p);
    } else {
        if (d->f32) hipLaunchKernelGGL((pw_wgrad_kernel<float, false>), grid, dim3(256), 0, s, p);
        else hipLaunchKernelGGL((pw_wgrad_kernel<bf16_t, false>), grid, dim3(256), 0, s, p);
    }
    return vg_check_launch();
}
```

van_gan_amd/csrc/vg_wgrad_dma.hip:

```cpp
#include "vg_dma_common.h"

__global__ __launch_bounds__(256) void materialize_kernel(const MatK p) {
    const int tid = threadIdx.x;
    int row = blockIdx.x;
    const int hp = row % p.Hp; row /= p.Hp;
    const int dp = row % p.Dp; const int n = row / p.Dp;
    int pd = dp + p.pmin_d, ph = hp + p.pmin_h;
    const int qd = pd + p.npad, qh = ph + p.npad;
    const bool vd = resolve_pos(pd, p.D, p.pad_mode), vh = resolve_pos(ph, p.H, p.pad_mode);
    const int npl = p.Cin >> 4;
    const int units = npl * p.Wps * 2;
    const int sh = p.shift0;
    const float slope = p.act == VG_ACT_RELU ? 0.f : (p.act == VG_ACT_LRELU ? VG_LRELU : 1.f);
    const int ND = p.D + 2 * p.npad, NH = p.H + 2 * p.npad, NW = p.W + 2 * p.npad;
    const bool nrow = p.noise && vd && vh && qd >= 0 && qd < ND && qh >= 0 && qh < NH;
    const size_t s0row = (((size_t)n * (p.D >> sh) + (pd >> sh)) * (p.H >> sh) + (ph >> sh)) * (p.W >> sh);
    const size_t s1row = (((size_t)n * p.D + pd) * p.H + ph) * p.W;
    const size_t nzrow = (((size_t)n * ND + (nrow ? qd : 0)) * NH + (nrow ? qh : 0)) * NW;
    for (int u = tid; u < units; u += 256) {
        const int plane = u / (p.Wps * 2), r = u - plane * p.Wps * 2;
        const int ws = r >> 1, half = r & 1;
        const int j = p.deint ? (ws < p.WE ? 2 * ws : 2 * (ws - p.WE) + 1) : ws;
        int pw = j + p.pmin_w;
        const int qw = pw + p.npad;
// ... 628 lines not shown
        if (do_db) {
            for (int v = db_v0; v < BM; v += db_vs) {
                const bf16x8 r = *(const bf16x8*)(yb + v * p.CO2 + db_s * 16);
#pragma unroll
                for (int e = 0; e < 8; ++e) dbs[e] += bf2f((bf16_t)r[e]);
            }
        }
        for (int ks = kgrp; ks < nks; ks += p.KS) {
            bf16x8 A[R], B[Q];
            const char* hk = hb + ks * 1024 + lx;
            const char* yk = yb + ks * ystep;
#pragma unroll
            for (int q = 0; q < Q; ++q) B[q] = tr_frag_d(yk + yq[q], yk + yq[q] + y16);
#pragma unroll
            for (int j = 0; j < R; ++j) A[j] = tr_frag_d(hk + poff[j], hk + poff[j] + 512);
#pragma unroll
            for (int j = 0; j < R; ++j)
#pragma unroll
                for (int q = 0; q < Q; ++q) acc[j][q] = VG_MFMA16(A[j], B[q], acc[j][q]);
        }
    }
    float* red = (float*)smem;
    int sl = 1;
    for (int step = 1; step < p.KS; step <<= 1, ++sl) {
        const int slot = rgrp * (p.KS >> sl) + (kgrp >> sl);
        __syncthreads();
        if ((kgrp & (2 * step - 1)) == step) {
            float* dst = red + (size_t)(slot * R * Q) * 256 + lane * 4;
#pragma unroll
            for (int j = 0; j < R; ++j)
#pragma unroll
                for (int q = 0; q < Q; ++q) *(f32x4*)(dst + (j * Q + q) * 256) = acc[j][q];
        }
        __syncthreads();
        if ((kgrp & (2 * step - 1)) == 0) {
            const float* src = red + (size_t)(slot * R * Q) * 256 + lane * 4;
#pragma unroll
            for (int j = 0; j < R; ++j)
#pragma unroll
                for (int q = 0; q < Q; ++q) acc[j][q] += *(const f32x4*)(src + (j * Q + q) * 256);
        }
    }
    if (kgrp == 0) {
#pragma unroll
        for (int j = 0; j < R; ++j) {
            const int pl = rgrp + p.RS * j;
            if (pl >= p.FA) continue;
            const int ci0 = pl * 16 + 4 * lg;
#pragma unroll
            for (int q = 0; q < Q; ++q) {
                const int co = cob * CO + q * 16 + li;
#pragma unroll
                for (int e = 0; e < 4; ++e) {
                    const size_t i = (size_t)(ci0 + e) * p.Cout + co;
                    if (p.part) p.part[(size_t)blockIdx.x * p.dw_elems + i] = acc[j][q][e];
                    else atomicAdd(&p.dw[i], acc[j][q][e]);
                }
            }
        }
    }
    if (do_db) {
        __syncthreads();
        if (tid < CO) red[tid] = 0.f;
        __syncthreads();
        if (db_v0 < BM) {
            const int fv = p.CO2 == 128 ? (db_v0 >> 1) & 3 : (p.CO2 == 64 ? (db_v0 >> 2) & 1 : 0);
            const int ch = 16 * ((db_s >> 1) ^ fv) + 8 * (db_s & 1);
#pragma unroll
            for (int e = 0; e < 8; ++e) atomicAdd(&red[ch + e], dbs[e]);
        }
        __syncthreads();
        if (tid < CO) atomicAdd(&p.db[cob * CO + tid], red[tid]);
    }
}

template <int R, int Q>
static void launch_wpw(const WpwK& k, dim3 grid, int lds, hipStream_t s) {
    static bool attr_set = false;
    if (!attr_set) {
        (void)hipFuncSetAttribute((const void*)wgrad_pw_dma_kernel<R, Q>, hipFuncAttributeMaxDynamicSharedMemorySize, VG_LDS_LIMIT);
        attr_set = true;
    }
    hipLaunchKernelGGL((wgrad_pw_dma_kernel<R, Q>), grid, dim3(512), lds, s, k);
}

int vg_wgrad_pw_dma(const vg_conv_desc* d, const void* dy, int dy_f32, int T_total, float* dw, float* db, float* scratch,
                    int64_t scratch_bytes, hipStream_t s) {
    if (!vg_tune("WGRAD_PW_DMA", 1)) return 1;
    const int Cin = d->c_src0 + d->c_src1;
    if (d->f32 || dy_f32 || d->src_f32 || d->wpack || d->ntaps != 1 || T_total != 1 || d->tap_d[0] || d->tap_h[0] || d->tap_w[0]) return 1;
    if (d->in_scale || d->act != VG_ACT_NONE || d->noise || !scratch) return 1;
    if (Cin < 16 || (Cin % 16) || (d->Cout % 16) || (d->c_src0 % 16) || (d->c_src1 % 16)) return 1;
    if (d->istr < 1 || d->istr > 2 || d->OD * d->istr != d->D || d->OH * d->istr != d->H || d->OW * d->istr != d->W) return 1;
    if (d->src0_shift && d->istr != 1) return 1;
    const int FA = Cin / 16;
    const int CO = d->Cout >= 64 ? 64 : d->Cout;
    if ((d->Cout % CO) || FA > 24) return 1;
    const int Q = CO / 16, ncob = d->Cout / CO;
    int R = 0, RS = 1;
    if (Q == 1) { R = 3; } else if (Q == 2) { R = 6; } else { R = FA <= 4 ? 4 : 6; }
    while (RS < 8 && RS * R < FA) RS <<= 1;
    if (RS * R < FA) return 1;
    const int KS = 8 / RS;
    int best[5] = {0, 0, 0, 0, 0};
    for (int bm = 512; bm >= 64 && !best[0]; bm >>= 1) {
        const int nA = FA * (bm / 32), nB = bm * CO * 2 / 1024;
        if (nA > 8 * VG_WD_MAXA || nB > 8 * VG_WD_MAXB || nB < 1) continue;
        const int bufb = (nA + nB) * 1024;
        if (2 * bufb > VG_LDS_LIMIT || (bm / 32) < KS) continue;
        if (8 * R * Q * 1024 / 2 > VG_LDS_LIMIT) continue;
        for (int tw = 16; tw >= 8 && !best[0]; tw >>= 1) {
            if (d->OW % tw) continue;
            for (int th = 2; th <= d->OH && tw * th <= bm; th <<= 1) {
                if ((d->OH % th) || tw * th < 32) continue;
                const int td = bm / (tw * th);
                if (td > d->OD || (d->OD % td) || (d->src0_shift && (td & 1))) continue;
                int nb = VG_LDS_LIMIT / bufb; if (nb > 4) nb = 4;
                best[0] = td; best[1] = th; best[2] = tw; best[3] = bufb; best[4] = nb;
                break;
            }
        }
    }
    if (!best[0]) return 1;
    const int TD = best[0], TH = best[1], TW = best[2], BM = TD * TH * TW;
    if (d->src0_shift && ((TD | TH | TW) & 1)) return 1;
    WpwK k;
    k.x0 = (const char*)d->src0; k.x1 = (const char*)d->src1; k.dy = (const char*)dy;
    k.c0 = d->c_src0; k.c1 = d->c_src1; k.sh0 = d->src0_shift ? 1 : 0; k.istr = d->istr;
    k.N = d->N; k.D = d->D; k.H = d->H; k.W = d->W; k.OD = d->OD; k.OH = d->OH; k.OW = d->OW; k.Cin = Cin; k.Cout = d->Cout;
    k.FA = FA; k.RS = RS; k.KS = KS; k.ksl = ilog2_exact(KS); k.ncob = ncob; k.CO2 = CO * 2; k.co2l = ilog2_exact(CO * 2);
    k.tdl = ilog2_exact(TD); k.thl = ilog2_exact(TH); k.twl = ilog2_exact(TW);
    k.tiles_d = d->OD / TD; k.tiles_h = d->OH / TH; k.tiles_w = d->OW / TW;
    k.total_tiles = d->N * k.tiles_d * k.tiles_h * k.tiles_w;
    k.ppp = BM / 32; k.nA = FA * k.ppp; k.nB = BM * CO * 2 / 1024; k.bufb = best[3]; k.nbuf = best[4];
    auto magic = [](int dd) { return dd <= 1 ? 0u : (unsigned)((1ULL << 32) / (unsigned)dd + 1ULL); };
    k.m_tpn = magic(k.tiles_d * k.tiles_h * k.tiles_w); k.m_tw = magic(k.tiles_w); k.m_th = magic(k.tiles_h); k.m_ppp = magic(k.ppp); k.m_ncob = magic(ncob);
    k.dw = dw; k.db = db; k.dw_elems = Cin * d->Cout;
    if ((int64_t)k.total_tiles * (k.total_tiles / d->N) >= (1LL << 32)) return 1;
    if (k.total_tiles * ncob < 32) return 1;
    int bx = vg_tune("WGRAD_PW_WGS", 256) / ncob; if (bx < 1) bx = 1; if (bx > k.total_tiles) bx = k.total_tiles;
    const int64_t part_bytes = (int64_t)bx * k.dw_elems * 4;
    if (part_bytes > scratch_bytes) return 1;
    k.part = (float*)scratch;
    int lds = k.nbuf * k.bufb; { const int rl = 4 * R * Q * 1024; if (rl > lds) lds = rl; }
    if (vg_dry("wgrad_pw_dma<%d,%d>|bm%d|rs%d|s%d|u%d|nb%d|walk%d", R, Q, BM, RS, d->istr, k.sh0, k.nbuf, k.total_tiles > bx ? 1 : 0)) return VG_OK;
    const dim3 grid(bx, ncob, 1);
    if (Q == 1) launch_wpw<3, 1>(k, grid, lds, s);
    else if (Q == 2) launch_wpw<6, 2>(k, grid, lds, s);
    else if (R == 4) launch_wpw<4, 4>(k, grid, lds, s);
    else launch_wpw<6, 4>(k, grid, lds, s);
    vg_launch_reduce_partials(k.part, bx, k.dw_elems, dw, s);
    return vg_check_launch();
}
```

van_gan_amd/nets.py:

```python
from __future__ import annotations

import math
import os
from typing import Dict, List, Optional, Tuple

import torch

from . import ops
from .ops import ACT_LRELU, ACT_NONE, ACT_RELU, Arena, ConvLayer, Src

GEN_F = [16, 32, 64, 128, 256]
_STEM_AUX = os.environ.get('VG_STEM_AUX', '1') != '0'
_STEM_FUSED = os.environ.get('VG_STEM_FUSED', '1') != '0'


def gen_param_specs(attention_gate: bool = False) -> List[Tuple[str, Tuple[int, ...], str]]:
    f = GEN_F
    s: List[Tuple[str, Tuple[int, ...], str]] = []

    def conv(name, k, ci, co, init):
        s.append((name + '.w', (k, k, k, ci, co), init)); s.append((name + '.b', (co,), 'zeros'))

    def inorm(name, c):
        s.append((name + '.gamma', (c,), 'ones')); s.append((name + '.beta', (c,), 'zeros'))
# ... 317 lines not shown
    def _block_fwd(self, ar: Arena, name: str, N: int, src_raw: Src, nrm_inputs, out_dims, co, ctx, save: bool = True, n1=None,
                   out_jobs=None, out: Optional[Act] = None):
        L, Nn = self.L, self.Nn
        mk = None
        if not save:
            if out is None:
                out = Act(ar, N, out_dims, co, dtype=self.dtype)
            mk = ar.mark()
        tail = n1 is not None
        if not tail:
            n1 = Nn[name + '.cb1'].finalize(ar, *nrm_inputs)
        s1 = Src(src_raw.x0, (N,) + tuple(L[name + '.cb1'].in_dims), src_raw.c0, src_raw.x1, src_raw.c1, src_raw.shift0,
                 scale=n1['scale'], shift=n1['shift'], act=ACT_RELU)
        r = Act(ar, N, out_dims, co, dtype=self.dtype)
        sc = Act(ar, N, out_dims, co, dtype=self.dtype)
        if tail:
            ns, n2 = Nn[name + '.short'].state(ar, N), Nn[name + '.cb2'].state(ar, N)
            f_s = ops.fin_desc(ar, sc.count, [Nn[name + '.short'].job(ns)])
            f_1 = ops.fin_desc(ar, r.count, [Nn[name + '.cb2'].job(n2)])
        fork = ops.fork_side()
        with fork:
            L[name + '.short'].forward(src_raw, sc.data, sums=sc.sums, fin=f_s if tail else None)
            if not tail:
                ns = Nn[name + '.short'].finalize(ar, sc)
        L[name + '.cb1'].forward(s1, r.data, sums=r.sums, fin=f_1 if tail else None)
        if not tail:
            n2 = Nn[name + '.cb2'].finalize(ar, r)
        fork.join()
        s2 = Src(r.data, (N,) + tuple(out_dims), co, scale=n2['scale'], shift=n2['shift'], act=ACT_RELU)
        if out is None:
            out = Act(ar, N, out_dims, co, dtype=self.dtype)
        f_o = ops.fin_desc(ar, out.count, out_jobs) if (tail and out_jobs) else None
        L[name + '.cb2'].forward(s2, out.data, sums=out.sums, res=sc.data, res_scale=ns['scale'], res_shift=ns['shift'], fin=f_o)
        if save:
            ctx[name] = dict(n1=n1, s1=s1, r=r, sc=sc, ns=ns, n2=n2, s2=s2, out=out, src_raw=src_raw)
        else:
            ar.release(mk)
        return out

    def forward(self, ar: Arena, x: torch.Tensor, y: torch.Tensor, save: bool = True) -> dict:
        return run_to_end(self.forward_iter(ar, x, y, save))

    def forward_iter(self, ar: Arena, x: torch.Tensor, y: torch.Tensor, save: bool = True):
        N = x.shape[0]
        f, lv, L, Nn = GEN_F, self.lv, self.L, self.Nn
        ctx = {'N': N, 'x': x, 'y': y}
        tail = ops.FIN_TAIL
        gate = self.attention_gate
        pre, jobs = {}, {}
        if tail:
            pre['stem.cb'], pre['stem.short'] = Nn['stem.cb'].state(ar, N), Nn['stem.short'].state(ar, N)
            for b in ['enc%d' % e for e in range(1, 5)] + ([] if gate else ['dec%d' % d for d in (3, 2, 1, 0)]):
                pre[b] = Nn[b + '.cb1'].state(ar, N)
            pre['bridge.cb1'], pre['bridge.cb2'] = Nn['bridge.cb1'].state(ar, N), Nn['bridge.cb2'].state(ar, N)
            dec_job = (lambda d, c_off=0: []) if gate else (lambda d, c_off=0: [Nn['dec%d.cb1' % d].job(pre['dec%d' % d], c_off)])
            jobs['stem'] = [Nn['enc1.cb1'].job(pre['enc1'])] + dec_job(0, f[1])
            for e in range(1, 4):
                jobs['enc%d' % e] = [Nn['enc%d.cb1' % (e + 1)].job(pre['enc%d' % (e + 1)])] + dec_job(e, f[e + 1])
            jobs['enc4'] = [Nn['bridge.cb1'].job(pre['bridge.cb1'])]
            jobs['bridge.cb1'] = [Nn['bridge.cb2'].job(pre['bridge.cb2'])]
            jobs['bridge.cb2'] = dec_job(3)
            for d in (3, 2, 1):
                jobs['dec%d' % d] = dec_job(d - 1)
            jobs['dec0'] = None
        sx = Src(x, (N,) + lv[0], 1, f32=True)
        c1 = Act(ar, N, lv[0], f[0], dtype=self.dtype)
        L['stem.conv1'].forward(sx, c1.data, sums=c1.sums, fin=ops.fin_desc(ar, c1.count, [Nn['stem.cb'].job(pre['stem.cb'])]) if tail else None)
        fused = _STEM_FUSED and _STEM_AUX
        if fused:
            sc = None
            ns = dict(scale=ar.alloc((N, f[0]), torch.float32), shift=ar.alloc((N, f[0]), torch.float32), mean=None, rstd=None, mult=None)
            ops.stem_short_fwd(ar, x, N, f[0], L['stem.short'].w, Nn['stem.short'].gamma, Nn['stem.short'].beta, ns['scale'], ns['shift'],
                               round16=self.dtype != torch.float32)
        else:
            sc = Act(ar, N, lv[0], f[0], dtype=self.dtype)
            L['stem.short'].forward(sx, sc.data, sums=sc.sums, fin=ops.fin_desc(ar, sc.count, [Nn['stem.short'].job(pre['stem.short'])]) if tail else None)
            ns = pre['stem.short'] if tail else Nn['stem.short'].finalize(ar, sc)
        n1 = pre['stem.cb'] if tail else Nn['stem.cb'].finalize(ar, c1)
        s1 = Src(c1.data, (N,) + lv[0], f[0], scale=n1['scale'], shift=n1['shift'], act=ACT_RELU)
        h = Act(ar, N, lv[0], f[0], dtype=self.dtype)
        L['stem.cb'].forward(s1, h.data, sums=h.sums, res=x if fused else sc.data, res_scale=ns['scale'], res_shift=ns['shift'],
                             fin=ops.fin_desc(ar, h.count, jobs['stem']) if tail else None, res_c1=fused)
        ctx['stem'] = dict(sx=sx, c1=c1, sc=sc, ns=ns, n1=n1, s1=s1, out=h)
        yield
        skips = [h]
        for e in range(1, 5):
            raw = Src(h.data, (N,) + lv[e - 1], f[e - 1])
            b = 'enc%d' % e
            h = self._block_fwd(ar, b, N, raw, (h,), lv[e], f[e], ctx, save, n1=pre.get(b), out_jobs=jobs.get(b))
            if save:
                ctx['enc%d' % e]['inp'] = (skips[-1],)
            skips.append(h)
            yield
        nb1 = pre['bridge.cb1'] if tail else Nn['bridge.cb1'].finalize(ar, h)
        sb1 = Src(h.data, (N,) + lv[4], f[4], scale=nb1['scale'], shift=nb1['shift'], act=ACT_RELU)
        b1 = Act(ar, N, lv[4], f[4], dtype=self.dtype)
        L['bridge.cb1'].forward(sb1, b1.data, sums=b1.sums, fin=ops.fin_desc(ar, b1.count, jobs['bridge.cb1']) if tail else None)
        nb2 = pre['bridge.cb2'] if tail else Nn['bridge.cb2'].finalize(ar, b1)
        sb2 = Src(b1.data, (N,) + lv[4], f[4], scale=nb2['scale'], shift=nb2['shift'], act=ACT_RELU)
        b2 = Act(ar, N, lv[4], f[4], dtype=self.dtype)
        L['bridge.cb2'].forward(sb2, b2.data, sums=b2.sums, fin=ops.fin_desc(ar, b2.count, jobs['bridge.cb2']) if (tail and jobs['bridge.cb2']) else None)
        ctx['bridge'] = dict(inp=h, nb1=nb1, sb1=sb1, b1=b1, nb2=nb2, sb2=sb2, b2=b2)
        h = b2
        for d in (3, 2, 1, 0):
            skip = skips[d]
            raw = Src(h.data, (N,) + lv[d], h.C, skip.data, skip.C, shift0=1)
            low = h
            yield
            b = 'dec%d' % d
            if self.attention_gate:
                out_pre = mkg = None
                if not save:
                    out_pre = Act(ar, N, lv[d], f[d], dtype=self.dtype)
                    mkg = ar.mark()
                gs, gctx = self._gate_fwd(ar, d, N, low, skip)
                raw = Src(low.data, (N,) + lv[d], low.C, gs.data, gs.C, shift0=1)
                n1 = Nn[b + '.cb1'].finalize(ar, low, gs) if tail else None
                h = self._block_fwd(ar, b, N, raw, (low, gs), lv[d], f[d], ctx, save, n1=n1, out_jobs=jobs.get(b), out=out_pre)
                if save:
                    ctx[b]['inp'] = (low, gs)
                    ctx[b]['gate'] = gctx
                else:
                    ar.release(mkg)
                continue
            h = self._block_fwd(ar, b, N, raw, (low, skip), lv[d], f[d], ctx, save, n1=pre.get(b), out_jobs=jobs.get(b))
            if save:
                ctx['dec%d' % d]['inp'] = (low, skip)
        so = Src(h.data, (N,) + lv[0], f[0])
        L['out'].forward(so, y, tanh=True)
        ctx['out'] = dict(so=so, inp=h)
        return ctx

    def _norm_desc(self, ar, g, g_padded, src: Src, st, norm: Norm, dx, act, dx_cstride=0, accumulate=True):
        N = src.N
        red = ops.alloc_red(ar, N, src.C)
        return ops.actnorm_desc(g, g_padded, src.x0, (N, src.D, src.H, src.W), src.C, dx, scale=st['scale'], shift=st['shift'],
                                act=act, norm=True, gamma=norm.gamma, mean=st['mean'], rstd=st['rstd'], red=red,
                                accumulate=accumulate, x1=src.x1, c_x0=src.c0 if src.x1 is not None else 0, x0_shift=src.shift0,
                                dx_cstride=dx_cstride, dgamma=norm.dgamma, dbeta=norm.dbeta)

    def _norm_bwd(self, ar, g, g_padded, src: Src, st, norm: Norm, dx, act, dx_cstride=0, accumulate=True):
        ops.actnorm_run(self._norm_desc(ar, g, g_padded, src, st, norm, dx, act, dx_cstride, accumulate))

    def _dgrad_norm_bwd(self, ar, lay, dy, N, dp, src: Src, st, norm: Norm, dx, act, accumulate):
        dsc = self._norm_desc(ar, dp, True, src, st, norm, dx, act, accumulate=accumulate)
        ops.actnorm_run(dsc, stats_done=lay.dgrad(dy, N, dp, accumulate=False, bstat=dsc))

    def _block_bwd(self, ar: Arena, name: str, c: dict, N: int, inline: bool = False):
        L, Nn = self.L, self.Nn
        out, r, sc = c['out'], c['r'], c['sc']
        d_out = out.grad
        cb1, cb2, short = L[name + '.cb1'], L[name + '.cb2'], L[name + '.short']
        mk = ar.mark()
        d_sc = ar.alloc(sc.data.shape, self.dtype)
        ssc = Src(sc.data, (N,) + sc.dims, sc.C)
        dsc1 = self._norm_desc(ar, d_out, False, ssc, c['ns'], Nn[name + '.short'], d_sc, ACT_NONE, accumulate=False)
        ops.actnorm_stats(dsc1)
        cb2.wgrad(c['s2'], d_out, inline)
        dp = ar.alloc((N,) + cb2.buf_dims + (r.C,), self.dtype)
        d_r = ar.alloc(r.data.shape, self.dtype)
        dsc2 = self._norm_desc(ar, dp, True, c['s2'], c['n2'], Nn[name + '.cb2'], d_r, ACT_RELU, accumulate=False)
        if not cb2.dgrad(d_out, N, dp, accumulate=False, bstat=dsc2):
            ops.actnorm_stats(dsc2)
        ops.actnorm_apply2(dsc1, dsc2)
        s1, raw = c['s1'], c['src_raw']
        cb1.wgrad(s1, d_r, inline)
        short.wgrad(raw, d_sc, inline)
        dp1 = ar.alloc((N,) + cb1.buf_dims + (s1.C,), self.dtype)
        inp = c['inp']
        if len(inp) == 1:
            gin = inp[0].alloc_grad(ar) if inp[0].grad is None else inp[0].grad
            assert inp[0].grad_init, 'encoder input gradient must have had its first (overwriting) writer: the decoder skip path'
            self._dgrad_norm_bwd(ar, cb1, d_r, N, dp1, s1, c['n1'], Nn[name + '.cb1'], gin, ACT_RELU, accumulate=True)
            short.dgrad(d_sc, N, gin, accumulate=True)
        else:
            low, skip = inp
            dsc = self._norm_desc(ar, dp1, True, s1, c['n1'], Nn[name + '.cb1'], None, ACT_RELU, accumulate=False)
            stats_done = cb1.dgrad(d_r, N, dp1, accumulate=False, bstat=dsc)
            if not stats_done:
                ops.actnorm_stats(dsc)
            a_low, a_skip = not low.first_write(), not skip.first_write()
            if not short.dgrad_concat_norm(d_sc, N, dsc, low.C, low.grad, skip.grad, acc_low=a_low, acc_skip=a_skip):
                dcat = ar.alloc((N,) + tuple(cb1.in_dims) + (s1.C,), self.dtype)
                ops.actnorm_set_dx(dsc, dcat)
                ops.actnorm_run(dsc, stats_done=True)
                short.dgrad_concat(d_sc, N, dcat, low.C, low.grad, skip.grad, acc_low=a_low, acc_skip=a_skip)
        ar.release(mk, defer=True)

    def backward(self, ar: Arena, ctx: dict, gy: torch.Tensor, inline_from: int = -1):
        run_to_end(self.backward_iter(ar, ctx, gy, inline_from))

    def grad_suffix_offset(self, first_param: str = 'enc4.cb1.in.gamma') -> int:
        return self.store.offsets[first_param][0]

    def backward_iter(self, ar: Arena, ctx: dict, gy: torch.Tensor, inline_from: int = -1, on_suffix_done=None):
        N = ctx['N']
        L, Nn = self.L, self.Nn
        acts = [ctx['stem']['out']] + [ctx['enc%d' % e]['out'] for e in range(1, 5)] + \
               [ctx['bridge']['b2']] + [ctx['dec%d' % d]['out'] for d in (3, 2, 1, 0)]
        if self.attention_gate:
            acts += [ctx['dec%d' % d]['inp'][1] for d in (3, 2, 1, 0)]
        for a in acts:
            a.grad = None
            a.alloc_grad(ar)
        dpre = ar.alloc(gy.shape, torch.float32)
        if isinstance(ctx['y'], list):
            nb = N // len(ctx['y'])
            for i, yi in enumerate(ctx['y']):
                ops.tanh_bwd(gy[i * nb:(i + 1) * nb], yi, dpre[i * nb:(i + 1) * nb])
        else:
            ops.tanh_bwd(gy, ctx['y'], dpre)
        h = ctx['out']['inp']
        L['out'].wgrad(ctx['out']['so'], dpre)
        L['out'].dgrad(dpre, N, h.grad, accumulate=not h.first_write())
        for d in (0, 1, 2, 3):
            self._block_bwd(ar, 'dec%d' % d, ctx['dec%d' % d], N)
            if self.attention_gate:
                self._gate_bwd(ar, d, ctx['dec%d' % d], N)
            yield
        b = ctx['bridge']
        mk = ar.mark()
        cb2, cb1 = L['bridge.cb2'], L['bridge.cb1']
        cb2.wgrad(b['sb2'], b['b2'].grad)
        dp = ar.alloc((N,) + cb2.buf_dims + (b['b1'].C,), self.dtype)
        d_b1 = ar.alloc(b['b1'].data.shape, self.dtype)
        self._dgrad_norm_bwd(ar, cb2, b['b2'].grad, N, dp, b['sb2'], b['nb2'], Nn['bridge.cb2'], d_b1, ACT_RELU, accumulate=False)
        cb1.wgrad(b['sb1'], d_b1)
        dp = ar.alloc((N,) + cb1.buf_dims + (b['inp'].C,), self.dtype)
        self._dgrad_norm_bwd(ar, cb1, d_b1, N, dp, b['sb1'], b['nb1'], Nn['bridge.cb1'], b['inp'].grad, ACT_RELU, accumulate=not b['inp'].first_write())
        ar.release(mk, defer=True)
        for e in (4, 3, 2, 1):
            yield
            self._block_bwd(ar, 'enc%d' % e, ctx['enc%d' % e], N, inline=e <= inline_from)
            if e == 4 and on_suffix_done is not None:
                on_suffix_done()
        yield
        inl = inline_from >= 0
        s = ctx['stem']
        d_out = s['out'].grad
        stem_aux = _STEM_AUX or s['sc'] is None
        ssc = None if s['sc'] is None else Src(s['sc'].data, (N,) + s['sc'].dims, s['sc'].C)
        if stem_aux:
            nrm = Nn['stem.short']
            ops.stem_short_bwd(ar, d_out, s['sx'].x0, N, GEN_F[0], L['stem.short'].w, nrm.gamma, L['stem.short'].gw,
                               dgamma=nrm.dgamma, dbeta=nrm.dbeta, round16=self.dtype != torch.float32)
        else:
            d_sc = ar.alloc(s['sc'].data.shape, self.dtype)
            self._norm_bwd(ar, d_out, False, ssc, s['ns'], Nn['stem.short'], d_sc, ACT_NONE, accumulate=False)
        cb = L['stem.cb']
        cb.wgrad(s['s1'], d_out, inl)
        dp = ar.alloc((N,) + cb.buf_dims + (s['c1'].C,), self.dtype)
        d_c1 = ar.alloc(s['c1'].data.shape, self.dtype)
        self._dgrad_norm_bwd(ar, cb, d_out, N, dp, s['s1'], s['n1'], Nn['stem.cb'], d_c1, ACT_RELU, accumulate=False)
        L['stem.conv1'].wgrad(s['sx'], d_c1, inl)
        if not stem_aux:
            L['stem.short'].wgrad(s['sx'], d_sc, inl)


RESNET_F, RESNET_DOWN, RESNET_RES, RESNET_UP = 32, 3, 6, 3


def resnet_param_specs() -> List[Tuple[str, Tuple[int, ...], str]]:
    s: List[Tuple[str, Tuple[int, ...], str]] = []

    def inorm(name, c):
        s.append((name + '.gamma', (c,), 'he_vec')); s.append((name + '.beta', (c,), 'zeros'))

    f = RESNET_F
    s.append(('c7.w', (7, 7, 7, 1, f), 'he_normal')); inorm('c7.in', f)
    for i in range(RESNET_DOWN):
        s.append(('down%d.w' % i, (3, 3, 3, f, 2 * f), 'he_normal')); inorm('down%d.in' % i, 2 * f)
        f *= 2
    for j in range(RESNET_RES):
        for c in ('c1', 'c2'):
            s.append(('res%d.%s.w' % (j, c), (3, 3, 3, f, f), 'he_normal')); inorm('res%d.%s.in' % (j, c), f)
    for i in range(RESNET_UP):
        s.append(('up%d.w' % i, (4, 4, 4, f, f // 2), 'he_normal')); inorm('up%d.in' % i, f // 2)
        f //= 2
    s.append(('out.w', (7, 7, 7, f, 1), 'glorot_uniform')); s.append(('out.b', (1,), 'zeros'))
    return s


class ResNetGenerator:

    def __init__(self, store: ParamStore, dims: Tuple[int, int, int], dtype: torch.dtype = torch.bfloat16):
        if any(n % 16 or n < 32 for n in dims):
            raise ValueError('spatial dims must be multiples of 16 and >= 32')
        self.dtype, self.store, self.dims = dtype, store, tuple(dims)
        L, Nn = {}, {}
        f = RESNET_F
        d = tuple(dims)
        L['c7'] = ConvLayer(store, 'c7', 7, 1, f, 1, 'reflect', False, d, need_dgrad=False, dtype=dtype)
        Nn['c7'] = Norm(store, 'c7.in', f)
        d = L['c7'].out_dims
        for i in range(RESNET_DOWN):
            k = 'down%d' % i
            L[k] = ConvLayer(store, k, 3, f, 2 * f, 2, 'reflect', False, d, need_dgrad=True, dtype=dtype)
            Nn[k] = Norm(store, k + '.in', 2 * f)
            d, f = L[k].out_dims, 2 * f
        for j in range(RESNET_RES):
            for c in ('c1', 'c2'):
                k = 'res%d.%s' % (j, c)
                L[k] = ConvLayer(store, k, 3, f, f, 1, 'reflect', False, d, need_dgrad=True, dtype=dtype)
                Nn[k] = Norm(store, k + '.in', f)
        for i in range(RESNET_UP):
            k = 'up%d' % i
            d = tuple(2 * n for n in d)
            L[k] = ConvLayer(store, k, 4, f, f // 2, 1, 'same', False, d, need_dgrad=True, dtype=dtype)
            Nn[k] = Norm(store, k + '.in', f // 2)
            f //= 2
        assert d == tuple(dims), (d, dims)
        self.head = [ConvLayer(store, 'out', 7, f, 1, 1, 'same', a == 0, d, need_dgrad=True, dtype=dtype,
                               tap_subset=list(range(a * 49, (a + 1) * 49))) for a in range(7)]
        self.L, self.Nn = L, Nn

    def pack(self):
        if getattr(self, '_ptab', None) is None:
            self._ptab = ops.PackTable(list(self.L.values()) + self.head, self.store.w.device)
        self._ptab.run()

    def forward(self, ar: Arena, x: torch.Tensor, y: torch.Tensor, drop: Optional[dict] = None, save: bool = True) -> dict:
        drop = drop or {}
        L, Nn = self.L, self.Nn
        N = x.shape[0]
        taps = {}
        ctx = {'N': N, 'y': y, 'chain': [], 'res': [], 'ups': []}
        h = Act(ar, N, L['c7'].out_dims, L['c7'].cout, dtype=self.dtype)
        src = Src(x, (N,) + self.dims, 1, f32=True)
        L['c7'].forward(src, h.data, sums=h.sums)
        taps['c7'] = h
        key = 'c7'
        ctx['c7'] = src
        for i in range(RESNET_DOWN):
            k = 'down%d' % i
            st = Nn[key].finalize(ar, h, mult=drop.get(key))
# ... 308 lines not shown
```

van_gan_amd/ops.py:

```python
from __future__ import annotations

import ctypes as C
import os
import math
from typing import List, Optional, Sequence, Tuple

import torch

from . import _lib
from ._lib import ACT_LRELU, ACT_NONE, ACT_RELU, PAD_REFLECT, PAD_ZERO, ActNormBwdDesc, ConvDesc, FinDesc, check, lib

IN_EPS = 1e-3
STRIPES = 8


def _p(t: Optional[torch.Tensor]) -> Optional[int]:
    return None if t is None else t.data_ptr()


def conv_variant(d) -> str:
    buf = C.create_string_buffer(512)
    _lib.lib.vg_conv3d_variant(C.byref(d), buf, 512)
    return buf.value.decode()

# ... 116 lines not shown

class Recorder:

    _PURE = DryRun._PASS + ('vg_conv3d_variant', 'vg_conv3d_wgrad_variant', 'vg_abi_sizeof', 'vg_version', 'vg_storage16')

    def __init__(self):
        self.cmds = []
        self.keep = []
        self._wrapped = {}

    def __getattr__(self, name):
        real = getattr(_lib.lib, name)
        if name in self._PURE:
            return real
        w = self._wrapped.get(name)
        if w is None:
            cmds = self.cmds

            def w(*a, _f=real):
                rc = _f(*a)
                cmds.append((_f, a))
                return rc
            self._wrapped[name] = w
        return w

    def __enter__(self):
        global REC, lib
        self._saved = lib
        REC, lib = self, self
        return self

    def __exit__(self, *exc):
        global REC, lib
        REC, lib = None, self._saved
        return False


REC: Optional[Recorder] = None


def _host(fn, *a):
    fn(*a)
    if REC is not None:
        REC.cmds.append((fn, a))


def wait_stream(waiter: torch.cuda.Stream, other: torch.cuda.Stream):
    if REC is None:
        waiter.wait_stream(other)
        return
    ev = torch.cuda.Event()
    _host(ev.record, other); _host(waiter.wait_event, ev)


def wait_event(waiter: torch.cuda.Stream, ev):
    _host(waiter.wait_event, ev)


def record_event(stream: torch.cuda.Stream):
    if REC is None:
        return stream.record_event()
    ev = torch.cuda.Event()
    _host(ev.record, stream)
    return ev


def zero_fill(t: torch.Tensor):
    if REC is None:
        t.zero_()
    else:
        check(lib.vg_memset_zero(_p(t), t.numel() * t.element_size(), stream()), 'vg_memset_zero')


def copy(dst: torch.Tensor, src: torch.Tensor):
    if REC is None or not (dst.is_contiguous() and src.is_contiguous() and dst.dtype == src.dtype and dst.numel() == src.numel()):
        assert REC is None, 'recorded copies must be contiguous and type-preserving'
        dst.copy_(src)
    else:
        check(lib.vg_copy_bytes(_p(dst), _p(src), dst.numel() * dst.element_size(), stream()), 'vg_copy_bytes')


class Fp16:

    def __enter__(self):
        global lib
        self._saved = lib
        lib = _lib.lib_fp16()
        return self

    def __exit__(self, *exc):
        global lib
        lib = self._saved
        return False


class KernelProfile:

    def __init__(self):
        self.rows = {}
        self.vrows = {}
        self.lrows = {}

    def begin(self):
        e = torch.cuda.Event(enable_timing=True)
        e.record()
        return e

    def end(self, kind: str, flops: float, e0, nbytes: float = 0.0, variant: Optional[str] = None, layer: Optional[str] = None):
        e1 = torch.cuda.Event(enable_timing=True)
        e1.record()
        r = self.rows.setdefault(kind, [0, 0.0, [], 0.0])
        r[0] += 1; r[1] += flops; r[2].append((e0, e1)); r[3] += nbytes
        if variant:
            tmpl = variant.split('|')[0].replace(',bs1>', ',bs>').replace(',bs2>', ',bs>').replace(',bs1,pl>', ',bs,pl>').replace(',bs2,pl>', ',bs,pl>')
            v = self.vrows.setdefault((kind, tmpl), [0, 0.0, [], 0.0])
            v[0] += 1; v[1] += flops; v[2].append((e0, e1)); v[3] += nbytes
            if layer:
                v = self.lrows.setdefault((kind, layer, tmpl), [0, 0.0, [], 0.0])
                v[0] += 1; v[1] += flops; v[2].append((e0, e1)); v[3] += nbytes

    def by_layer(self):
        torch.cuda.synchronize()
        rows = []
        for (kind, layer, var), (n, fl, evs, nb) in self.lrows.items():
            ms = sum(a.elapsed_time(b) for a, b in evs)
            rows.append(dict(kind=kind, layer=layer, kernel=var, launches=n, ms=ms, gflop=fl / 1e9,
                             tflops=fl / (ms * 1e-3) / 1e12 if ms > 0 else None, algorithmic_bytes=nb))
        return sorted(rows, key=lambda r: -r['ms'])

    def summary(self):
        torch.cuda.synchronize()
        out = {}
        for k, (n, fl, evs, nb) in self.rows.items():
            ms = sum(a.elapsed_time(b) for a, b in evs)
            out[k] = dict(launches=n, flops=fl, ms=ms, bytes=nb)
        return out

    def by_variant(self):
        torch.cuda.synchronize()
        rows = []
        for (kind, var), (n, fl, evs, nb) in self.vrows.items():
            ms = sum(a.elapsed_time(b) for a, b in evs)
            rows.append(dict(kind=kind, kernel=var, launches=n, ms=ms, gflop=fl / 1e9, tflops=fl / (ms * 1e-3) / 1e12 if ms > 0 else None,
                             algorithmic_bytes=nb))
        return sorted(rows, key=lambda r: -r['ms'])


PROF: Optional[KernelProfile] = None

LAZY_RELEASE = os.environ.get('VG_LAZY_RELEASE', '1') != '0'
FORK_SHORT = os.environ.get('VG_FORK_SHORT', '1') != '0'
FUSE_CONCAT_NORM = os.environ.get('VG_FUSE_CONCAT_NORM', '1') != '0'
FUSE_CONCAT = os.environ.get('VG_FUSE_CONCAT', '1') != '0'
BSTAT = os.environ.get('VG_BSTAT', '1') != '0'
BSTAT_DMA = os.environ.get('VG_BSTAT_DMA', '0') != '0'
SIDE: Optional[bool] = None
_SIDE_OF = {}


def side_enable(device, on: bool = True):
    global SIDE
    SIDE = True if on else None


def _side_key(cur: torch.cuda.Stream):
    return (cur.device.index, cur.cuda_stream)


def _side_of(cur: torch.cuda.Stream) -> torch.cuda.Stream:
    sd = _SIDE_OF.get(_side_key(cur))
    if sd is None:
        sd = _SIDE_OF[_side_key(cur)] = torch.cuda.Stream(device=cur.device)
    return sd


class fork_side:

    def __init__(self):
        self.on = SIDE is not None and PROF is None and DRY is None and FORK_SHORT
        self.cur = self.sd = self.ctx = None

    def __enter__(self):
        if self.on:
            self.cur = current_stream_obj()
            self.sd = _side_of(self.cur)
            wait_stream(self.sd, self.cur)
            self.ctx = torch.cuda.stream(self.sd)
            self.ctx.__enter__()
        return self

    def __exit__(self, *exc):
        if self.on:
            self.ctx.__exit__(*exc)
        return False

    def join(self):
        if self.on:
            wait_stream(self.cur, self.sd)


def side_event():
    if SIDE is None:
        return None
    sd = _SIDE_OF.get(_side_key(current_stream_obj()))
    return None if sd is None else record_event(sd)


def side_join():
    if SIDE is not None:
        cur = current_stream_obj()
        sd = _SIDE_OF.get(_side_key(cur))
        if sd is not None:
            wait_stream(cur, sd)


CONV_SCRATCH = {}
CONV_SCRATCH_BYTES = _lib.SCRATCH_CTR_BYTES + (int(os.environ.get('VG_CONV_SCRATCH_MB', '160')) << 20)
_SCRATCH_RETIRED = []


def conv_scratch(d: ConvDesc, s_: int, device=None):
    need = CONV_SCRATCH_BYTES
    if d.wlayout:
        need = max(need, int(lib.vg_conv3d_scratch_bytes(C.byref(d))))
    if DRY is not None:
        d.scratch, d.scratch_bytes = 1 << 20, need
        return
    key = (_DEV if device is None else device, s_)
    sc = CONV_SCRATCH.get(key)
    if sc is None or sc.numel() < need:
        dev = torch.device('cuda', key[0]) if key[0] is not None else torch.device('cuda')
        if sc is not None:
            _SCRATCH_RETIRED.append(sc)
        sc = torch.empty(need, dtype=torch.uint8, device=dev)
        sc[:_lib.SCRATCH_CTR_BYTES].zero_()
        CONV_SCRATCH[key] = sc
    d.scratch, d.scratch_bytes = sc.data_ptr(), sc.numel()


WGRAD_SCRATCH = {}
WGRAD_SCRATCH_ELEMS = 96 << 20


class Arena:
    ZPOOL = 8 << 20

    def __init__(self, nbytes: int, device):
        self.buf = torch.empty(nbytes + self.ZPOOL, dtype=torch.uint8, device=device)
        self.zpool = self.buf[nbytes:]
        self.buf = self.buf[:nbytes]
        self.off = 0
        self.zoff = 0
        self.peak = 0
        self.lazy_ok = True
        self.zpool.zero_()
        self._pair, self._pairs, self._pair_pos, self._full = None, {}, {}, {}
        self._cache, self._cpos, self._halves = [], 0, {}

    def pair_begin(self, key, slot: int):
        self._pair = (key, slot)
        self._pair_pos[key] = 0
        if slot == 0:
            self._pairs[key] = []

    def pair_resume(self, key, slot: int):
        self._pair = (key, slot)

    def pair_end(self):
        self._pair = None

    def full_of(self, t):
        return None if t is None else self._full.get(t.data_ptr())

    def reset(self):
        self._pair, self._pairs, self._pair_pos, self._full = None, {}, {}, {}
        self._cpos = 0
        self.off = 0
        self.zmax = max(getattr(self, 'zmax', 0), self.zoff)
        nz = self.zoff if REC is None else self.ZPOOL
        if nz:
            zero_fill(self.zpool[:nz])
        self.zoff = 0

    _ESZ = {torch.float32: 4, torch.bfloat16: 2, torch.float16: 2, torch.int32: 4, torch.int64: 8, torch.uint8: 1, torch.float64: 8}

    def alloc(self, shape: Sequence[int], dtype: torch.dtype, zero: bool = False) -> torch.Tensor:
        shape = tuple(shape)
        if self._pair is not None and not zero:
            key, slot = self._pair
            if slot == 0:
                self._pair = None
                full = self.alloc((2 * shape[0],) + shape[1:], dtype)
                self._pair = (key, slot)
                self._pairs[key].append(full)
                self._full[full.data_ptr()] = full
                h = self._halves.get(full.data_ptr())
                if h is None or h[0] is not full:
                    h = self._halves[full.data_ptr()] = (full, full[:shape[0]], full[shape[0]:])
                return h[1]
            full = self._pairs[key][self._pair_pos[key]]
            self._pair_pos[key] += 1
            assert tuple(full.shape) == (2 * shape[0],) + shape[1:] and full.dtype == dtype, 'paired allocation sequences differ'
            return self._halves[full.data_ptr()][2]
        i, cache = self._cpos, self._cache
        if i < len(cache):
            e = cache[i]
# ... 404 lines not shown
        d.c_src0, d.c_src1, d.src0_shift = self.cout, 0, 0
        d.src_f32 = 0 if probe else int(dy.dtype == torch.float32 and self.cout == 1)
        d.N = N
        d.D, d.H, d.W = self.out_dims
        d.act, d.istr, d.pad_mode = ACT_NONE, 1, PAD_ZERO
        taps = [t for c in self.d_classes for t in c['taps']]
        _set_taps(d, taps)
        d.OD, d.OH, d.OW = [max(c['iters'][a] for c in self.d_classes) for a in range(3)]
        d.ostr = self.stride
        d.ooff_d, d.ooff_h, d.ooff_w = self.d_classes[0]['off']
        d.BD, d.BH, d.BW = self.buf_dims
        d.Cout, d.CK = self.cin, self.d_classes[0]['ck']
        d.f32 = self.f32
        d.nclass = len(self.d_classes)
        t0 = 0
        for i, c in enumerate(self.d_classes):
            d.cls_tap0[i] = t0
            t0 += len(c['taps'])
            d.cls_w[i] = dummy if probe else c['wp'].data_ptr()
            for a in range(3):
                d.cls_ooff[i][a] = c['off'][a]
                d.cls_iters[i][a] = c['iters'][a]
        d.cls_tap0[len(self.d_classes)] = t0
        d.wpacked = d.cls_w[0]
        d.wlayout = getattr(self, 'd_bn', 0)
        if probe and not plan:
            return d
        if probe:
            d.out = dummy
            plan = (C.c_int32 * 4)()
            ok = lib.vg_conv3d_plan(C.byref(d), plan) == 0
            self._last_plan = tuple(plan)
            return d if ok else None
        d.out, d.out_f32, d.accumulate = _p(out), int(out.dtype == torch.float32), int(accumulate)
        return d

    def dgrad(self, dy: torch.Tensor, N: int, out: torch.Tensor, accumulate: bool, bstat=None, bias=None) -> bool:
        use_bs = bstat is not None and BSTAT and not accumulate and not self.f32 and out.dtype in (torch.bfloat16, torch.float16) and bstat.norm \
            and ((len(self.d_classes) == 1 and self.stride == 1 and self.k == 3 and self.pad == 'reflect'
                  and self.d_classes[0]['ck'] == 16 and self.cin % 16 == 0 and self.cout % 16 == 0 and not bstat.mult)
                 or (bool(self.d_bn) and BSTAT_DMA))
        if DRY is not None:
            DRY.tag = ('dgrad', self.name)
            DRY.recipe = dict(kind='dgrad', layer=self.ctor, N=N, accumulate=bool(accumulate), dy_f32=dy.dtype == torch.float32,
                              out_f32=out.dtype == torch.float32, bstat=None if not use_bs else dict(
                                  cat=bool(bstat.x1), c_x0=bstat.c_x0, act=bstat.act, pad=bool(bstat.g_padded), mult=bool(bstat.mult),
                                  alias_n0=bstat.alias_n0, alias_shift=bstat.alias_shift))
        if REC is not None and use_bs:
            REC.keep.append(bstat)
        if self.d_fused:
            t = getattr(self, '_dg_tmpl', None)
            if t is None:
                t = self._dg_tmpl = self._fused_desc(dy, N, out, accumulate)
            d = ConvDesc()
            C.memmove(C.byref(d), C.byref(t), C.sizeof(ConvDesc))
            d.src0, d.N = _p(dy), N
            d.src_f32 = int(dy.dtype == torch.float32 and self.cout == 1)
            d.out, d.out_f32, d.accumulate = _p(out), int(out.dtype == torch.float32), int(accumulate)
            d.bstat = C.addressof(bstat) if use_bs else None
            d.bias = _p(bias)
            s_ = stream()
            conv_scratch(d, s_, out.device.index)
            e0 = PROF.begin() if PROF is not None else None
            check(lib.vg_conv3d(C.byref(d), s_), 'vg_conv3d(dgrad, fused classes) ' + self.name)
            if e0 is not None:
                PROF.end('conv_dgrad', 2.0 * N * math.prod(self.out_dims) * self.cin * self.cout * self.k ** 3, e0,
                         N * 2 * (math.prod(self.out_dims) * self.cout + math.prod(self.buf_dims) * self.cin), conv_variant(d), self.name)
            return use_bs
        for c in self.d_classes:
            t = c.get('tmpl')
            if t is None:
                t = ConvDesc()
                t.src1 = None
                t.c_src0, t.c_src1, t.src0_shift = self.cout, 0, 0
                t.D, t.H, t.W = self.out_dims
                t.act, t.istr, t.pad_mode = ACT_NONE, 1, PAD_ZERO
                _set_taps(t, c['taps'])
                t.OD, t.OH, t.OW = c['iters']
                t.ostr = self.stride
                t.ooff_d, t.ooff_h, t.ooff_w = c['off']
                t.BD, t.BH, t.BW = self.buf_dims
                t.Cout, t.wpacked, t.CK = self.cin, _p(c['wp']), c['ck']
                t.f32 = self.f32
                c['tmpl'] = t
            d = ConvDesc()
            C.memmove(C.byref(d), C.byref(t), C.sizeof(ConvDesc))
            d.src0, d.N = _p(dy), N
            d.src_f32 = int(dy.dtype == torch.float32 and self.cout == 1)
            d.out, d.out_f32, d.accumulate = _p(out), int(out.dtype == torch.float32), int(accumulate)
            d.bstat = C.addressof(bstat) if use_bs else None
            d.bias = _p(bias)
            s_ = stream()
            conv_scratch(d, s_, out.device.index)
            e0 = PROF.begin() if PROF is not None else None
            check(lib.vg_conv3d(C.byref(d), s_), 'vg_conv3d(dgrad) ' + self.name)
            if e0 is not None:
                PROF.end('conv_dgrad', 2.0 * N * math.prod(self.out_dims) * self.cin * self.cout * len(c['taps']), e0,
                         N * (4 if self.f32 else 2) * (math.prod(self.out_dims) * self.cout * len(c['taps']) / self.k ** 3
                                                       + math.prod(c['iters']) * self.cin), conv_variant(d), self.name)
        return use_bs


    def _sc_desc(self, dy, N):
        c = self.d_classes[0]
        d = ConvDesc()
        d.src1 = None
        d.c_src0, d.c_src1, d.src0_shift = self.cout, 0, 0
        d.D, d.H, d.W = self.out_dims
        d.act, d.istr, d.pad_mode = ACT_NONE, 1, PAD_ZERO
        _set_taps(d, c['taps'])
        d.OD, d.OH, d.OW = c['iters']
        d.ostr = self.stride
        d.ooff_d, d.ooff_h, d.ooff_w = c['off']
        d.BD, d.BH, d.BW = self.buf_dims
        d.Cout, d.wpacked, d.CK = self.cin, _p(c['wp']), c['ck']
        d.f32 = self.f32
        d.src0, d.N = _p(dy), N
        return d

    def dgrad_input(self, ar: 'Arena', dy: torch.Tensor, N: int, dx: torch.Tensor):
        assert self.cin == 1 and self.pad == 'reflect'
        if self.cell is None or DRY is not None or dy.dtype not in (torch.bfloat16, torch.float16):
            dp = ar.alloc((N,) + tuple(self.buf_dims) + (1,), self.dtype)
            self.dgrad(dy, N, dp, accumulate=False)
            actnorm_bwd(dp, True, None, (N,) + tuple(self.in_dims), 1, dx, act=ACT_NONE, norm=False, accumulate=False)
            return
        c = self.cell
        cells = ar.alloc((N,) + c['dims'] + (16,), self.dtype)
        t = c.get('tmpl')
        if t is None:
            t = c['tmpl'] = ConvDesc()
            t.src1 = None
            t.c_src0, t.c_src1, t.src0_shift = self.cout, 0, 0
            t.D, t.H, t.W = self.out_dims
            t.act, t.istr, t.pad_mode, t.ostr = ACT_NONE, 1, PAD_ZERO, 1
            _set_taps(t, c['taps'])
            t.OD, t.OH, t.OW = c['dims']
            t.BD, t.BH, t.BW = c['dims']
            t.Cout, t.wpacked, t.CK = 16, _p(c['wp']), 16
            t.f32 = 0
        d = ConvDesc()
        C.memmove(C.byref(d), C.byref(t), C.sizeof(ConvDesc))
        d.src0, d.N, d.out = _p(dy), N, _p(cells)
        s_ = stream()
        conv_scratch(d, s_, dy.device.index)
        e0 = PROF.begin() if PROF is not None else None
        check(lib.vg_conv3d(C.byref(d), s_), 'vg_conv3d(dgrad, cells) ' + self.name)
        if e0 is not None:
            PROF.end('conv_dgrad', 2.0 * N * math.prod(self.out_dims) * self.cin * self.cout * self.k ** 3, e0,
                     N * 2 * (math.prod(self.out_dims) * self.cout + math.prod(c['dims']) * 16), conv_variant(d), self.name)
        D_, H_, W_ = self.in_dims
        check(lib.vg_cells_fold(_p(cells), N, D_, H_, W_, _p(dx), s_), 'vg_cells_fold ' + self.name)

    def dgrad_concat_norm(self, dy: torch.Tensor, N: int, nd: 'ActNormBwdDesc', c_low: int, dlow: torch.Tensor, dskip: torch.Tensor,
                          acc_low: bool, acc_skip: bool) -> bool:
        if not (FUSE_CONCAT and FUSE_CONCAT_NORM and DRY is None and not self.f32 and self.k == 1 and self.stride == 1
                and len(self.d_classes) == 1 and not self.d_fused):
            return False
        c = self.d_classes[0]
        d = self._sc_desc(dy, N)
        e0 = PROF.begin() if PROF is not None else None
        rc = lib.vg_shortcut_dgrad_concat_norm(C.byref(d), C.byref(nd), _p(dlow), _p(dskip), c_low,
                                               int(bool(acc_low)) | (int(bool(acc_skip)) << 1), stream())
        if rc < 0:
            check(rc, 'vg_shortcut_dgrad_concat_norm ' + self.name)
        if rc == 0 and e0 is not None:
            PROF.end('conv_dgrad', 2.0 * N * math.prod(c['iters']) * self.cin * self.cout, e0,
                     N * 2 * (math.prod(self.out_dims) * self.cout + math.prod(self.buf_dims) * self.cin),
                     'pw_gemm_split<%d,%d,n1>' % ((self.cout + 31) // 32, self.cin // 16), self.name)
        return rc == 0

    def dgrad_concat(self, dy: torch.Tensor, N: int, dcat: torch.Tensor, c_low: int, dlow: torch.Tensor, dskip: torch.Tensor,
                     acc_low: bool, acc_skip: bool):
        fused = (FUSE_CONCAT and DRY is None and not self.f32 and self.k == 1 and self.stride == 1 and len(self.d_classes) == 1
                 and not self.d_fused and dcat.dtype == torch.bfloat16)
        if fused:
            c = self.d_classes[0]
            d = ConvDesc()
            d.src1 = None
            d.c_src0, d.c_src1, d.src0_shift = self.cout, 0, 0
            d.D, d.H, d.W = self.out_dims
            d.act, d.istr, d.pad_mode = ACT_NONE, 1, PAD_ZERO
            _set_taps(d, c['taps'])
            d.OD, d.OH, d.OW = c['iters']
            d.ostr = self.stride
            d.ooff_d, d.ooff_h, d.ooff_w = c['off']
            d.BD, d.BH, d.BW = self.buf_dims
            d.Cout, d.wpacked, d.CK = self.cin, _p(c['wp']), c['ck']
            d.f32 = self.f32
            d.src0, d.N = _p(dy), N
            d.out, d.out_f32, d.accumulate = _p(dcat), 0, 1
            e0 = PROF.begin() if PROF is not None else None
            rc = lib.vg_shortcut_dgrad_concat(C.byref(d), _p(dlow), _p(dskip), c_low, int(bool(acc_low)) | (int(bool(acc_skip)) << 1), stream())
            if rc == 0:
                if e0 is not None:
                    PROF.end('conv_dgrad', 2.0 * N * math.prod(c['iters']) * self.cin * self.cout, e0,
                             N * 2 * (math.prod(self.out_dims) * self.cout + math.prod(self.buf_dims) * self.cin),
                             'pw_gemm_split<%d,%d,n0>' % ((self.cout + 31) // 32, self.cin // 16), self.name)
                return
            if rc < 0:
                check(rc, 'vg_shortcut_dgrad_concat ' + self.name)
        self.dgrad(dy, N, dcat, accumulate=True)
        concat_bwd(dcat, (N,) + tuple(self.in_dims), c_low, self.cin - c_low, dlow, dskip, acc_low=acc_low, acc_skip=acc_skip)


class ConvTranspose3dK2S2:

    def __init__(self, store, name: str, cin: int, filters: int, in_dims: Tuple[int, int, int], dtype: torch.dtype = torch.bfloat16):
        self.cin, self.filters, self.in_dims, self.out_dims = cin, filters, tuple(in_dims), tuple(2 * n for n in in_dims)
        self.conv = ConvLayer(store, name, 2, filters, cin, 2, 'same', False, self.out_dims, need_dgrad=True, dtype=dtype)
        self.b, self.gb = store.param(name + '.b'), store.grad(name + '.b')

    def pack(self):
        self.conv.pack()

    def forward(self, x: torch.Tensor, N: int, out: torch.Tensor):
        assert tuple(x.shape) == (N,) + self.in_dims + (self.cin,) and tuple(out.shape) == (N,) + self.out_dims + (self.filters,)
        self.conv.dgrad(x, N, out, accumulate=False, bias=self.b)

    def backward(self, x: torch.Tensor, dy: torch.Tensor, N: int, dx: Optional[torch.Tensor]):
        src = Src(dy, (N,) + self.out_dims, self.filters, f32=False)
        if dx is not None:
            self.conv.forward(src, dx)
        self.conv.wgrad(src, x)
        check(lib.vg_bias_grad(_p(dy), int(dy.dtype == torch.float32), N * math.prod(self.out_dims), self.filters, _p(self.gb), stream()),
              'vg_bias_grad')


class PackTable:

    def __init__(self, layers, device):
        items = [it for l in layers for it in l.pack_items()]
        arr = (_lib.PackItem * len(items))()
        blk = 0
        per_block = int(os.environ.get('VG_PACK_ELEMS', 8192))
        for a, (w, idx, out, cin, cout, ntaps, tr, ck, f32, bn) in zip(arr, items):
            a.w, a.tap_idx, a.out = w.data_ptr(), idx.data_ptr(), out.data_ptr()
            a.Cin, a.Cout, a.ntaps, a.transpose, a.CK, a.out_f32, a.bn = cin, cout, ntaps, tr, ck, f32, bn
            a.blk0, a.nblk = blk, max(1, min(4096, -(-out.numel() // per_block)))
            blk += a.nblk
        self.total_blocks = blk
        raw = bytes(arr)
        self.keep = items
        self.n = len(items)
        self.table = torch.frombuffer(bytearray(raw), dtype=torch.uint8).to(device)
        self.cells = [l for l in layers if getattr(l, 'cell', None) is not None]
        self.ups = [l for l in layers if getattr(l, 'wp_up', None) is not None]

    def run(self):
        check(lib.vg_pack_weights_multi(_p(self.table), self.n, self.total_blocks, stream()), 'vg_pack_weights_multi')
        for l in self.cells:
            l.pack_cell()
        for l in self.ups:
            l.pack_up()


class SpecNormTable:

    def __init__(self, ws, us, device):
        assert 0 < len(ws) == len(us) <= 8
        arr = (_lib.SnItem * len(ws))()
        self.state = torch.zeros(len(ws), _lib.SN_STATE, dtype=torch.float32, device=device)
        blk = 0
        for i, (a, w, u) in enumerate(zip(arr, ws, us)):
            cout = w.shape[-1]
            K = w.numel() // cout
            nblk = _lib.lib.vg_spectral_norm_blocks(K, cout)
            if (nblk < 1 or w.dtype != torch.float32 or u.dtype != torch.float32 or u.numel() != cout or not w.is_contiguous()
                    or not u.is_contiguous() or (w.data_ptr() | u.data_ptr()) & 15):
                raise ValueError('vg_spectral_norm does not serve a [%d, %d] kernel (Cout in 64/128/256/512, K * Cout a multiple of 256, '
                                 'contiguous 16-byte aligned fp32)' % (K, cout))
            a.w, a.u, a.state = w.data_ptr(), u.data_ptr(), self.state[i].data_ptr()
            a.K, a.Cout, a.blk0, a.nblk = K, cout, blk, nblk
            blk += nblk
        self.total_blocks, self.n = blk, len(ws)
        self.keep = (list(ws), list(us))
        self.table = torch.frombuffer(bytearray(bytes(arr)), dtype=torch.uint8).to(device)
        self.scratch = torch.empty(_lib.lib.vg_spectral_norm_scratch_bytes(blk) // 4, dtype=torch.float32, device=device)

    def run(self, n_proj: int = 1):
        check(lib.vg_spectral_norm(_p(self.table), self.n, self.total_blocks, n_proj, _p(self.scratch), self.scratch.numel() * 4, stream()),
              'vg_spectral_norm')


def in_finalize(sums0, c0, count0, gamma, beta, N, scale, shift, mean=None, rstd=None, sums1=None, c1=0, count1=1.0,
                mult=None):
    check(lib.vg_in_finalize(_p(sums0), c0, float(count0), _p(sums1), c1, float(count1), _p(gamma), _p(beta), _p(mult),
                             N, IN_EPS, _p(scale), _p(shift), _p(mean), _p(rstd), stream()), 'vg_in_finalize')


FIN_TAIL = os.environ.get('VG_FIN_TAIL', '1') != '0'


def fin_desc(ar: 'Arena', count: float, jobs) -> FinDesc:
    f = FinDesc()
    tk = ar.alloc((1,), torch.int32, zero=True)
    f.ticket, f.count, f.eps, f.njobs = _p(tk), float(count), IN_EPS, len(jobs)
    keep = [tk]
    for j, (gamma, beta, mult, st, c_off, c_tot) in enumerate(jobs):
        q = f.job[j]
        q.gamma, q.beta, q.mult = _p(gamma), _p(beta), _p(mult)
        q.scale, q.shift, q.mean, q.rstd = _p(st['scale']), _p(st['shift']), _p(st['mean']), _p(st['rstd'])
        q.c_off, q.c_tot = c_off, c_tot
        keep += [gamma, beta, mult, st]
    f._keep = keep
    return f


def alloc_red(ar: 'Arena', N: int, C_: int) -> torch.Tensor:
    return ar.alloc((STRIPES * N * C_ * 2 + 4,), torch.float32, zero=True)


def actnorm_desc(g, g_padded, x, dims, C_, dx, *, scale=None, shift=None, mult=None, act=ACT_NONE, norm=False,
                 gamma=None, mean=None, rstd=None, red=None, accumulate=False, x1=None, c_x0=0, x0_shift=0,
                 dx_cstride=0, dx_coff=0, dgamma=None, dbeta=None, alias_n0=0, alias_shift=0, pgrad_n=0) -> ActNormBwdDesc:
    d = ActNormBwdDesc()
    d.g, d.g_padded = _p(g), int(g_padded)
    d.x, d.x_f32 = _p(x), int(x is not None and x.dtype == torch.float32)
    d.x1, d.c_x0, d.x0_shift = _p(x1), c_x0, x0_shift
    d.N, d.D, d.H, d.W = dims
    d.C = C_
    d.scale, d.shift, d.mult, d.act, d.norm = _p(scale), _p(shift), _p(mult), act, int(norm)
# ... 194 lines not shown
```

Before: 124.2 Mvoxels/s.

## Compute shortcut instance-norm backward from GEMM moments instead of materializing d_sc

For the concat-input residual shortcut (1x1 conv followed by instance norm), a new kernel accumulates second-order moments (x^T dy, x^T x, row sums) in one pass. From these it derives the weight, gamma and beta gradients and per-channel affine coefficients analytically. The dgrad GEMM then rebuilds the normalized gradient on the fly as a*g + b*sx + c, instead of first writing a d_sc tensor via actnorm stats/apply and running a separate shortcut wgrad. This removes a full-resolution intermediate and two passes, but adds the Cin^2 moment MFMA work, a partial-sum reduction, a finalize kernel, and bf16 rounding of the recomposed gradient.

```diff
diff --git a/include/vangan_hip.h b/include/vangan_hip.h
--- a/include/vangan_hip.h
+++ b/include/vangan_hip.h
@@ -166,6 +166,11 @@
 int vg_shortcut_dgrad_concat_norm(const vg_conv_desc* d, const vg_actnorm_bwd_desc* b, void* dlow, void* dskip, int c_low,
                                   int accumulate, vg_stream_t stream);
 
+int vg_shortcut_moments(const vg_conv_desc* d, const void* g, const float* w, const float* gamma, const float* mean, const float* rstd,
+                        int round16, float* dw, float* dgamma, float* dbeta, float* coef, vg_stream_t stream);
+int vg_shortcut_dgrad_concat_norm_affine(const vg_conv_desc* d, const vg_actnorm_bwd_desc* b, const void* sx, const float* coef,
+                                         void* dlow, void* dskip, int c_low, int accumulate, vg_stream_t stream);
+
 int vg_affine_add(const void* a, const float* a_scale, const float* a_shift, int a_act, const void* b, const float* b_scale,
                   const float* b_shift, int N, int64_t S, int C, void* out, int f32, vg_stream_t stream);
 
diff --git a/van_gan_amd/_lib.py b/van_gan_amd/_lib.py
--- a/van_gan_amd/_lib.py
+++ b/van_gan_amd/_lib.py
@@ -104,6 +104,10 @@
     'vg_concat_bwd': ([c_void_p, c_int, c_int, c_int, c_int, c_int, c_int, c_void_p, c_void_p, c_int, c_int, c_void_p], c_int),
     'vg_shortcut_dgrad_concat': ([C.POINTER(ConvDesc), c_void_p, c_void_p, c_int, c_int, c_void_p], c_int),
     'vg_shortcut_dgrad_concat_norm': ([C.POINTER(ConvDesc), C.POINTER(ActNormBwdDesc), c_void_p, c_void_p, c_int, c_int, c_void_p], c_int),
+    'vg_shortcut_moments': ([C.POINTER(ConvDesc), c_void_p, c_void_p, c_void_p, c_void_p, c_void_p, c_int, c_void_p, c_void_p, c_void_p, c_void_p,
+                             c_void_p], c_int),
+    'vg_shortcut_dgrad_concat_norm_affine': ([C.POINTER(ConvDesc), C.POINTER(ActNormBwdDesc), c_void_p, c_void_p, c_void_p, c_void_p, c_int, c_int,
+                                              c_void_p], c_int),
     'vg_affine_add': ([c_void_p, c_void_p, c_void_p, c_int, c_void_p, c_void_p, c_void_p, c_int, c_i64, c_int, c_void_p, c_int, c_void_p], c_int),
     'vg_bias_grad': ([c_void_p, c_int, c_i64, c_int, c_void_p, c_void_p], c_int),
     'vg_pack_cell_weights': ([c_void_p, c_int, c_void_p, c_void_p], c_int),
diff --git a/van_gan_amd/csrc/vg_pointwise.hip b/van_gan_amd/csrc/vg_pointwise.hip
--- a/van_gan_amd/csrc/vg_pointwise.hip
+++ b/van_gan_amd/csrc/vg_pointwise.hip
@@ -203,6 +203,7 @@
     const float* n_scale; const float* n_shift; const float* n_mean; const float* n_rstd; const float* n_gamma; const float* n_mult;
     VgFin fin;
     const float* n_red; float* n_dgamma; float* n_dbeta; int n_act;
+    const bf16_t* sx; const float* coef;
 };
 }
 extern unsigned long long* g_vg_stamps;
@@ -258,6 +259,13 @@
             ntab_s[3 * C + tid] = k1 - cc * mu;
             ntab_s[4 * C + tid] = cc;
         }
+    }
+    __shared__ float ctab[SPLIT == 2 ? 3 * KS * 32 : 1];
+    if constexpr (SPLIT == 2) {
+        if (p.coef && tid < p.Cin) {
+            const float* cf = p.coef + ((size_t)n * p.Cin + tid) * 3;
+            ctab[tid] = cf[0]; ctab[KS * 32 + tid] = cf[1]; ctab[2 * KS * 32 + tid] = cf[2];
+        }
         __syncthreads();
     }
     bf16x8 wA[NB][KS];
@@ -306,6 +314,7 @@
     };
     for (int wt = blockIdx.x * 4 + wave; wt < nwt; wt += gridDim.x * 4) {
         bf16x8 xb[MS][KS];
+        Raw8<bf16_t> xs[SPLIT == 2 ? MS : 1][SPLIT == 2 ? KS : 1];
         bool vok[MS], oks[MS / 2];
         size_t i0s[MS], i1s[MS], ovs[MS / 2];
         size_t ovf[MS / 2];
@@ -361,6 +370,7 @@
                 raw_load(t, q);
                 raw_mask(t, cok);
                 xb[i][ks] = t.v;
+                if constexpr (SPLIT == 2) { if (p.coef) raw_load(xs[i][ks], p.sx + i0s[i] * p.c0 + ce); }
             }
         if (p.stamps) { asm volatile("s_waitcnt vmcnt(0)" ::: "memory"); if (lane == 0) p.stamps[((size_t)blockIdx.x * 4 + wave) * 8 + 2] = __builtin_amdgcn_s_memrealtime(); }
         if constexpr (SPLIT == 2) {
@@ -385,6 +395,23 @@
                     raw_load(gq[nb][jh], p.ng + gi[jh] + nb * 16);
                     raw_load(xq[nb][jh], nb * 16 < p.sc0 ? p.nx0 + li[jh] + nb * 16 : p.nx1 + si[jh] + (nb * 16 - p.sc0));
                 }
+            if (p.coef) {
+#pragma unroll
+                for (int i = 0; i < MS; ++i)
+#pragma unroll
+                    for (int ks = 0; ks < KS; ++ks) {
+                        const int c = ks * 32 + kg * 8;
+                        const bool cok = c < p.Cin;
+                        const float* ct = ctab + (cok ? c : c % p.Cin);
+                        Raw8<bf16_t> t; t.v = xb[i][ks];
+                        float gv[8], sv[8];
+                        raw_unpack(t, gv); raw_unpack(xs[i][ks], sv);
+#pragma unroll
+                        for (int e = 0; e < 8; ++e) t.v[e] = (short)f2bf(ct[e] * gv[e] + ct[KS * 32 + e] * sv[e] + ct[2 * KS * 32 + e]);
+                        raw_mask(t, cok);
+                        xb[i][ks] = t.v;
+                    }
+            }
 #pragma unroll
             for (int nb = 0; nb < NB; ++nb) {
                 f32x4 a[MS];
@@ -915,7 +942,8 @@
     return ok ? vg_check_launch() : 1;
 }
 
-int pw_gemm_split(const vg_conv_desc* d, const vg_actnorm_bwd_desc* nb_, void* dlow, void* dskip, int c_low, int acc, hipStream_t s) {
+int pw_gemm_split(const vg_conv_desc* d, const vg_actnorm_bwd_desc* nb_, void* dlow, void* dskip, int c_low, int acc, hipStream_t s,
+                  const void* sx = nullptr, const float* coef = nullptr) {
     if (!pw_enabled() || !vg_tune("PW_GEMM", 1) || !vg_tune("PW_SPLIT", 1)) return 1;
     if (d->ntaps != 1 || d->tap_d[0] || d->tap_h[0] || d->tap_w[0] || d->noise || d->wpack || d->nclass > 1) return 1;
     if (d->f32 || d->src_f32 || d->out_f32 || d->in_scale || d->act != VG_ACT_NONE || d->res || d->tanh_out || d->out_sums || d->bias) return 1;
@@ -945,6 +973,7 @@
         p.ng = (const bf16_t*)nb_->g; p.nx0 = (const bf16_t*)nb_->x; p.nx1 = (const bf16_t*)nb_->x1;
         p.n_scale = nb_->scale; p.n_shift = nb_->shift; p.n_mean = nb_->mean; p.n_rstd = nb_->rstd; p.n_gamma = nb_->gamma; p.n_mult = nb_->mult;
         p.n_red = nb_->red; p.n_dgamma = (nb_->dgamma && nb_->dbeta) ? nb_->dgamma : nullptr; p.n_dbeta = nb_->dbeta; p.n_act = nb_->act;
+        p.sx = (const bf16_t*)sx; p.coef = sx ? coef : nullptr;
     }
     const int MS = (KS * NB <= 2) ? 4 : 2;
     const int64_t nwt = (SO + MS * 16 - 1) / (MS * 16);
@@ -1005,6 +1034,14 @@
     return pw_gemm_split(d, b, dlow, dskip, c_low, accumulate, (hipStream_t)stream);
 }
 
+extern "C" int vg_shortcut_dgrad_concat_norm_affine(const vg_conv_desc* d, const vg_actnorm_bwd_desc* b, const void* sx, const float* coef,
+                                                    void* dlow, void* dskip, int c_low, int accumulate, vg_stream_t stream) {
+    vg_begin();
+    if (!d || !b || !d->src0 || !d->wpacked || !dlow || !dskip || !sx || !coef) return VG_EINVAL;
+    if (!vg_tune("PW_SPLIT_NORM", 1) || !vg_tune("SHORTCUT_MOMENTS", 1) || vg_dry_on()) return 1;
+    return pw_gemm_split(d, b, dlow, dskip, c_low, accumulate, (hipStream_t)stream, sx, coef);
+}
+
 int vg_pointwise_conv(const vg_conv_desc* d, hipStream_t s) {
     if (pw_enabled() && !d->res && !d->tanh_out && !d->accumulate && d->ostr == 1 && !d->ooff_d && !d->ooff_h && !d->ooff_w
         && d->BD == d->OD && d->BH == d->OH && d->BW == d->OW && !(d->out_f32 && !d->f32)) {
diff --git a/van_gan_amd/csrc/vg_wgrad_dma.hip b/van_gan_amd/csrc/vg_wgrad_dma.hip
--- a/van_gan_amd/csrc/vg_wgrad_dma.hip
+++ b/van_gan_amd/csrc/vg_wgrad_dma.hip
@@ -804,3 +804,294 @@
     vg_launch_reduce_partials(k.part, bx, k.dw_elems, dw, s);
     return vg_check_launch();
 }
+
+template <int R, int Q, int RS, int MINB>
+__global__ __launch_bounds__(512, MINB) void shortcut_moments_kernel(const WpwK p) {
+    extern __shared__ __attribute__((aligned(16))) char smem[];
+    const int tid = threadIdx.x, lane = tid & 63;
+    const int wave = __builtin_amdgcn_readfirstlane(tid >> 6);
+    const int lg = lane >> 4, li = lane & 15;
+    const int n = blockIdx.y;
+    constexpr int KS = 8 / RS, RW = R / RS;
+    const int kgrp = wave & (KS - 1), rgrp = wave / KS;
+    const int BM = 1 << (p.tdl + p.thl + p.twl);
+    const int nks = BM >> 5;
+    const int TWm = (1 << p.twl) - 1, THm = (1 << p.thl) - 1;
+    const int Hs = p.H >> p.sh0, Ws = p.W >> p.sh0;
+    int aoffs[VG_WD_MAXA], boffs[VG_WD_MAXB];
+#pragma unroll
+    for (int k = 0; k < VG_WD_MAXA; ++k) {
+        const int piece = wave + 8 * k;
+        const int plane = fast_div(piece, p.m_ppp), pk = piece - plane * p.ppp;
+        const int m = pk * 32 + (lane >> 1);
+        const int c = plane * 16 + (lane & 1) * 8;
+        const int w = m & TWm, h = (m >> p.twl) & THm, d = m >> (p.twl + p.thl);
+        aoffs[k] = c < p.c0 ? ((((d >> p.sh0) * Hs + (h >> p.sh0)) * Ws + (w >> p.sh0)) * p.c0 + c) * 2
+                            : (((d * p.H + h) * p.W + w) * p.c1 + (c - p.c0)) * 2;
+    }
+#pragma unroll
+    for (int k = 0; k < VG_WD_MAXB; ++k) {
+        const int byte = (wave + 8 * k) * 1024 + lane * 16;
+        int m = byte >> p.co2l; const int s = (byte - (m << p.co2l)) >> 4;
+        if (m >= BM) m = 0;
+        const int f = p.CO2 == 64 ? (m >> 2) & 1 : 0;
+        const int blk = (s >> 1) ^ f;
+        const int w = m & TWm, h = (m >> p.twl) & THm, d = m >> (p.twl + p.thl);
+        boffs[k] = (((d * p.OH + h) * p.OW + w) * p.Cout + blk * 16 + (s & 1) * 8) * 2;
+    }
+    const unsigned lds0 = (unsigned)(uintptr_t)(lds_void_d*)smem;
+    auto issue = [&](int tile, int bufoff) {
+        const int t1 = fast_div(tile, p.m_tw), ti_w = tile - t1 * p.tiles_w;
+        const int ti_d = fast_div(t1, p.m_th), ti_h = t1 - ti_d * p.tiles_h;
+        const int d0 = ti_d << p.tdl, h0 = ti_h << p.thl, w0 = ti_w << p.twl;
+        const char* a0 = p.x0 + ((((size_t)n * (p.D >> p.sh0) + (d0 >> p.sh0)) * Hs + (h0 >> p.sh0)) * Ws + (w0 >> p.sh0)) * p.c0 * 2;
+        const char* a1 = p.x1 + ((((size_t)n * p.D + d0) * p.H + h0) * p.W + w0) * p.c1 * 2;
+        const char* bbase = p.dy + ((((size_t)n * p.OD + d0) * p.OH + h0) * p.OW + w0) * p.Cout * 2;
+#pragma unroll
+        for (int k = 0; k < VG_WD_MAXA; ++k) {
+            const int piece = wave + 8 * k;
+            if (piece < p.nA) {
+                const bool lo = fast_div(piece, p.m_ppp) * 16 < p.c0;
+                glds16(lo ? a0 : a1, aoffs[k], lds0 + bufoff + piece * 1024);
+            }
+        }
+#pragma unroll
+        for (int k = 0; k < VG_WD_MAXB; ++k) {
+            const int piece = wave + 8 * k;
+            if (piece < p.nB) glds16(bbase, boffs[k], lds0 + bufoff + (p.nA + piece) * 1024);
+        }
+    };
+    const int ntw = ((int)blockIdx.x < p.total_tiles) ? (p.total_tiles - (int)blockIdx.x + (int)gridDim.x - 1) / (int)gridDim.x : 0;
+    const int n_w = (wave < p.nA ? (p.nA - wave + 7) >> 3 : 0) + (wave < p.nB ? (p.nB - wave + 7) >> 3 : 0);
+    for (int j = 0; j < p.nbuf - 1 && j < ntw; ++j) issue(blockIdx.x + j * gridDim.x, j * p.bufb);
+
+    constexpr int NC = Q + R + 1, NF = RW * NC + Q, FD = RW * NC;
+    f32x4 acc[NF];
+#pragma unroll
+    for (int f = 0; f < NF; ++f) acc[f] = (f32x4){0.f, 0.f, 0.f, 0.f};
+    const short one = (short)f2bf(1.f);
+    const bf16x8 ones = (bf16x8){one, one, one, one, one, one, one, one};
+    const int m0l = 4 * lg + (li >> 2);
+    const int fsw = p.CO2 == 64 ? (m0l >> 2) & 1 : 0;
+    int yq[Q];
+#pragma unroll
+    for (int q = 0; q < Q; ++q) yq[q] = m0l * p.CO2 + 32 * (q ^ fsw) + 8 * (li & 3);
+    const int lx = m0l * 32 + 8 * (li & 3);
+    const int ystep = 32 * p.CO2, y16 = 16 * p.CO2;
+    const int pstride = BM * 32;
+
+    int cur = 0, nxt = p.nbuf - 1;
+    for (int it = 0; it < ntw; ++it) {
+        const char* hb = smem + cur * p.bufb;
+        const int newer = min(p.nbuf - 2, ntw - 1 - it);
+        wait_vmcnt(newer * n_w);
+        __syncthreads();
+        if (it + p.nbuf - 1 < ntw) issue(blockIdx.x + (it + p.nbuf - 1) * gridDim.x, nxt * p.bufb);
+        cur = cur + 1 == p.nbuf ? 0 : cur + 1; nxt = nxt + 1 == p.nbuf ? 0 : nxt + 1;
+        const char* yb = hb + p.nA * 1024;
+        for (int ks = kgrp; ks < nks; ks += KS) {
+            bf16x8 A[R], B[Q];
+            const char* hk = hb + ks * 1024 + lx;
+            const char* yk = yb + ks * ystep;
+#pragma unroll
+            for (int q = 0; q < Q; ++q) B[q] = tr_frag_d(yk + yq[q], yk + yq[q] + y16);
+#pragma unroll
+            for (int j = 0; j < R; ++j) A[j] = tr_frag_d(hk + j * pstride, hk + j * pstride + 512);
+#pragma unroll
+            for (int j = 0; j < RW; ++j) {
+                bf16x8 Aj = A[j];
+                if (RS > 1) {
+#pragma unroll
+                    for (int g = 1; g < RS; ++g) if (rgrp == g) Aj = A[g * RW + j];
+                }
+#pragma unroll
+                for (int q = 0; q < Q; ++q) acc[j * NC + q] = VG_MFMA16(Aj, B[q], acc[j * NC + q]);
+#pragma unroll
+                for (int i = 0; i < R; ++i) acc[j * NC + Q + i] = VG_MFMA16(Aj, A[i], acc[j * NC + Q + i]);
+                acc[j * NC + Q + R] = VG_MFMA16(Aj, ones, acc[j * NC + Q + R]);
+            }
+#pragma unroll
+            for (int q = 0; q < Q; ++q) acc[FD + q] = VG_MFMA16(ones, B[q], acc[FD + q]);
+        }
+    }
+    constexpr int SL = (3 * RS * NF <= 160) ? 3 : ((2 * RS * NF <= 160) ? 2 : 1);
+    float* red = (float*)smem;
+    for (int base = 1; base < KS; base += SL) {
+        __syncthreads();
+        if (kgrp >= base && kgrp < base + SL) {
+            float* dst = red + (size_t)(((kgrp - base) * RS + rgrp) * NF) * 256 + lane * 4;
+#pragma unroll
+            for (int f = 0; f < NF; ++f) *(f32x4*)(dst + f * 256) = acc[f];
+        }
+        __syncthreads();
+        if (kgrp == 0) {
+            for (int s = 0; s < SL && base + s < KS; ++s) {
+                const float* src = red + (size_t)((s * RS + rgrp) * NF) * 256 + lane * 4;
+#pragma unroll
+                for (int f = 0; f < NF; ++f) acc[f] += *(const f32x4*)(src + f * 256);
+            }
+        }
+    }
+    if (kgrp != 0) return;
+    float* out = p.part + ((size_t)n * gridDim.x + blockIdx.x) * p.dw_elems;
+    float* oQ = out + p.Cin * p.Cout; float* oR = oQ + p.Cin * p.Cin; float* oD = oR + p.Cin;
+#pragma unroll
+    for (int j = 0; j < RW; ++j) {
+        const int ci0 = (rgrp * RW + j) * 16 + 4 * lg;
+#pragma unroll
+        for (int e = 0; e < 4; ++e) {
+#pragma unroll
+            for (int q = 0; q < Q; ++q) out[(size_t)(ci0 + e) * p.Cout + q * 16 + li] = acc[j * NC + q][e];
+#pragma unroll
+            for (int i = 0; i < R; ++i) oQ[(size_t)(ci0 + e) * p.Cin + i * 16 + li] = acc[j * NC + Q + i][e];
+            if (li == 0) oR[ci0 + e] = acc[j * NC + Q + R][e];
+        }
+    }
+    if (rgrp == 0 && lg == 0) {
+#pragma unroll
+        for (int q = 0; q < Q; ++q) oD[q * 16 + li] = acc[FD + q][0];
+    }
+}
+
+__global__ __launch_bounds__(256) void shortcut_moments_sum_kernel(const float* __restrict__ part, int nb, int E, double* __restrict__ mom) {
+    const int e = blockIdx.x * 256 + threadIdx.x, n = blockIdx.y;
+    if (e >= E) return;
+    const float* q = part + (size_t)n * nb * E + e;
+    double s = 0.0;
+    int b = 0;
+    for (; b + 8 <= nb; b += 8) {
+        float v[8];
+#pragma unroll
+        for (int k = 0; k < 8; ++k) v[k] = q[(size_t)(b + k) * E];
+#pragma unroll
+        for (int k = 0; k < 8; ++k) s += (double)v[k];
+    }
+    for (; b < nb; ++b) s += (double)q[(size_t)b * E];
+    mom[(size_t)n * E + e] = s;
+}
+
+struct ScFinK {
+    const double* mom; const float* w; const float* gamma; const float* mean; const float* rstd;
+    float* dw; float* dgamma; float* dbeta; float* coef;
+    int N, Cin, Cout, round16; double S;
+};
+__global__ __launch_bounds__(128) void shortcut_finalize_kernel(const ScFinK p) {
+    __shared__ double wc[128], term[128];
+    const int c = blockIdx.x, i = threadIdx.x;
+    const bool on = i < p.Cin;
+    const int E = p.Cin * p.Cout + p.Cin * p.Cin + p.Cin + p.Cout;
+    float wf = on ? p.w[(size_t)i * p.Cout + c] : 0.f;
+    if (p.round16) wf = bfround(wf);
+    wc[i] = (double)wf;
+    __syncthreads();
+    double dwi = 0.0, dg = 0.0, db = 0.0;
+    for (int n = 0; n < p.N; ++n) {
+        const double* G = p.mom + (size_t)n * E; const double* Qm = G + p.Cin * p.Cout; const double* r = Qm + p.Cin * p.Cin;
+        const double D1 = r[p.Cin + c];
+        double gc = 0.0, cw = 0.0;
+        if (on) {
+            const double mi = r[i] / p.S;
+            gc = G[(size_t)i * p.Cout + c] - mi * D1;
+            for (int j = 0; j < p.Cin; ++j) cw += (Qm[(size_t)i * p.Cin + j] - mi * r[j]) * wc[j];
+        }
+        __syncthreads();
+        term[i] = wc[i] * gc;
+        __syncthreads();
+        double d2 = 0.0;
+        for (int j = 0; j < p.Cin; ++j) d2 += term[j];
+        const int nc = n * p.Cout + c;
+        const double rho = (double)p.rstd[nc], mu = (double)p.mean[nc];
+        d2 *= rho;
+        const double k0 = (double)p.gamma[c] * rho, k1 = k0 * D1 / p.S, k2 = k0 * d2 / p.S;
+        dwi += k0 * gc - k2 * rho * cw;
+        if (i == 0) {
+            dg += d2; db += D1;
+            p.coef[(size_t)nc * 3] = (float)k0; p.coef[(size_t)nc * 3 + 1] = (float)(-k2 * rho); p.coef[(size_t)nc * 3 + 2] = (float)(k2 * rho * mu - k1);
+        }
+    }
+    if (on) atomicAdd(&p.dw[(size_t)i * p.Cout + c], (float)dwi);
+    if (i == 0) {
+        if (p.dgamma) atomicAdd(&p.dgamma[c], (float)dg);
+        if (p.dbeta) atomicAdd(&p.dbeta[c], (float)db);
+    }
+}
+
+template <int R, int Q, int RS, int MINB>
+static void launch_scm(const WpwK& k, dim3 grid, int lds, hipStream_t s) {
+    static bool attr_set = false;
+    if (!attr_set) {
+        (void)hipFuncSetAttribute((const void*)shortcut_moments_kernel<R, Q, RS, MINB>, hipFuncAttributeMaxDynamicSharedMemorySize, VG_LDS_LIMIT);
+        attr_set = true;
+    }
+    hipLaunchKernelGGL((shortcut_moments_kernel<R, Q, RS, MINB>), grid, dim3(512), lds, s, k);
+}
+
+extern "C" int vg_shortcut_moments(const vg_conv_desc* d, const void* g, const float* w, const float* gamma, const float* mean,
+                                   const float* rstd, int round16, float* dw, float* dgamma, float* dbeta, float* coef, vg_stream_t stream) {
+    vg_begin();
+    if (!d || !d->src0 || !g || !w || !gamma || !mean || !rstd || !dw || !coef) return VG_EINVAL;
+    if (!vg_tune("SHORTCUT_MOMENTS", 1)) return 1;
+    hipStream_t s = (hipStream_t)stream;
+    const int Cin = d->c_src0 + d->c_src1;
+    if (d->f32 || d->src_f32 || d->wpack || d->ntaps != 1 || d->tap_d[0] || d->tap_h[0] || d->tap_w[0]) return 1;
+    if (d->in_scale || d->act != VG_ACT_NONE || d->noise || !d->scratch || !d->src1) return 1;
+    if (Cin < 16 || (Cin % 16) || (d->Cout % 16) || (d->c_src0 % 16) || (d->c_src1 % 16) || d->c_src1 < 16) return 1;
+    if (d->istr != 1 || d->OD != d->D || d->OH != d->H || d->OW != d->W || d->N < 1) return 1;
+    if (!vg_tune("PW", 1) || !vg_tune("PW_GEMM", 1) || !vg_tune("PW_SPLIT", 1) || !vg_tune("PW_SPLIT_NORM", 1)) return 1;
+    const int FA = Cin / 16, Q = d->Cout / 16;
+    if (!((FA == 3 && Q == 1) || (FA == 6 && Q == 2))) return 1;
+    const int RS = FA == 3 ? 1 : 2, KS = 8 / RS;
+    const int NF = (FA / RS) * (Q + FA + 1) + Q, SL = (3 * RS * NF <= 160) ? 3 : ((2 * RS * NF <= 160) ? 2 : 1);
+    int best[5] = {0, 0, 0, 0, 0};
+    for (int bm = 512; bm >= 32 * KS && !best[0]; bm >>= 1) {
+        const int nA = FA * (bm / 32), nB = bm * d->Cout * 2 / 1024;
+        if (nA > 8 * VG_WD_MAXA || nB > 8 * VG_WD_MAXB || nB < 1) continue;
+        const int bufb = (nA + nB) * 1024;
+        if (2 * bufb > VG_LDS_LIMIT) continue;
+        for (int tw = 16; tw >= 8 && !best[0]; tw >>= 1) {
+            if (d->OW % tw) continue;
+            for (int th = 2; th <= d->OH && tw * th <= bm; th <<= 1) {
+                if ((d->OH % th) || tw * th < 32) continue;
+                const int td = bm / (tw * th);
+                if (td > d->OD || (d->OD % td) || (d->src0_shift && (td & 1))) continue;
+                int nb = VG_LDS_LIMIT / bufb; if (nb > 4) nb = 4;
+                best[0] = td; best[1] = th; best[2] = tw; best[3] = bufb; best[4] = nb;
+                break;
+            }
+        }
+    }
+    if (!best[0]) return 1;
+    const int TD = best[0], TH = best[1], TW = best[2], BM = TD * TH * TW;
+    if (d->src0_shift && (((TD | TH | TW) & 1) || ((d->D | d->H | d->W) & 1))) return 1;
+    WpwK k = {};
+    k.x0 = (const char*)d->src0; k.x1 = (const char*)d->src1; k.dy = (const char*)g;
+    k.c0 = d->c_src0; k.c1 = d->c_src1; k.sh0 = d->src0_shift ? 1 : 0; k.istr = 1;
+    k.N = d->N; k.D = d->D; k.H = d->H; k.W = d->W; k.OD = d->OD; k.OH = d->OH; k.OW = d->OW; k.Cin = Cin; k.Cout = d->Cout;
+    k.FA = FA; k.RS = RS; k.KS = KS; k.ksl = ilog2_exact(KS); k.ncob = 1; k.CO2 = d->Cout * 2; k.co2l = ilog2_exact(k.CO2);
+    k.tdl = ilog2_exact(TD); k.thl = ilog2_exact(TH); k.twl = ilog2_exact(TW);
+    k.tiles_d = d->OD / TD; k.tiles_h = d->OH / TH; k.tiles_w = d->OW / TW;
+    k.total_tiles = k.tiles_d * k.tiles_h * k.tiles_w;
+    k.ppp = BM / 32; k.nA = FA * k.ppp; k.nB = BM * d->Cout * 2 / 1024; k.bufb = best[3]; k.nbuf = best[4];
+    auto magic = [](int dd) { return dd <= 1 ? 0u : (unsigned)((1ULL << 32) / (unsigned)dd + 1ULL); };
+    k.m_tw = magic(k.tiles_w); k.m_th = magic(k.tiles_h); k.m_ppp = magic(k.ppp);
+    if ((int64_t)k.total_tiles * k.total_tiles >= (1LL << 32)) return 1;
+    if (k.total_tiles < 32) return 1;
+    const int E = Cin * d->Cout + Cin * Cin + Cin + d->Cout;
+    k.dw_elems = E;
+    int bx = vg_tune("SHORTCUT_MOMENTS_WGS", 256) / d->N; if (bx < 1) bx = 1; if (bx > k.total_tiles) bx = k.total_tiles;
+    const int64_t part_bytes = (int64_t)d->N * bx * E * 4, mom_bytes = (int64_t)d->N * E * 8;
+    if (VG_SCRATCH_CTR_BYTES + part_bytes + mom_bytes > d->scratch_bytes) return 1;
+    if (vg_dry_on()) return 1;
+    k.part = (float*)((char*)d->scratch + VG_SCRATCH_CTR_BYTES);
+    double* mom = (double*)((char*)k.part + part_bytes);
+    int lds = k.nbuf * k.bufb; { const int rl = SL * RS * NF * 1024; if (rl > lds) lds = rl; }
+    if (lds > VG_LDS_LIMIT) return 1;
+    const dim3 grid(bx, d->N, 1);
+    if (Q == 1) launch_scm<3, 1, 1, 2>(k, grid, lds, s); else launch_scm<6, 2, 2, 1>(k, grid, lds, s);
+    hipLaunchKernelGGL(shortcut_moments_sum_kernel, dim3((E + 255) / 256, d->N), dim3(256), 0, s, k.part, bx, E, mom);
+    ScFinK f;
+    f.mom = mom; f.w = w; f.gamma = gamma; f.mean = mean; f.rstd = rstd; f.dw = dw; f.dgamma = dgamma; f.dbeta = dbeta; f.coef = coef;
+    f.N = d->N; f.Cin = Cin; f.Cout = d->Cout; f.round16 = round16; f.S = (double)d->OD * d->OH * d->OW;
+    hipLaunchKernelGGL(shortcut_finalize_kernel, dim3(d->Cout), dim3(128), 0, s, f);
+    return vg_check_launch();
+}
diff --git a/van_gan_amd/nets.py b/van_gan_amd/nets.py
--- a/van_gan_amd/nets.py
+++ b/van_gan_amd/nets.py
@@ -493,20 +493,29 @@
         d_out = out.grad
         cb1, cb2, short = L[name + '.cb1'], L[name + '.cb2'], L[name + '.short']
         mk = ar.mark()
-        d_sc = ar.alloc(sc.data.shape, self.dtype)
-        ssc = Src(sc.data, (N,) + sc.dims, sc.C)
-        dsc1 = self._norm_desc(ar, d_out, False, ssc, c['ns'], Nn[name + '.short'], d_sc, ACT_NONE, accumulate=False)
-        ops.actnorm_stats(dsc1)
+        coef = None
+        if len(c['inp']) == 2:
+            nsh = Nn[name + '.short']
+            coef = short.shortcut_moments(ar, c['src_raw'], d_out, nsh.gamma, c['ns'], nsh.dgamma, nsh.dbeta)
+        if coef is None:
+            d_sc = ar.alloc(sc.data.shape, self.dtype)
+            ssc = Src(sc.data, (N,) + sc.dims, sc.C)
+            dsc1 = self._norm_desc(ar, d_out, False, ssc, c['ns'], Nn[name + '.short'], d_sc, ACT_NONE, accumulate=False)
+            ops.actnorm_stats(dsc1)
         cb2.wgrad(c['s2'], d_out, inline)
         dp = ar.alloc((N,) + cb2.buf_dims + (r.C,), self.dtype)
         d_r = ar.alloc(r.data.shape, self.dtype)
         dsc2 = self._norm_desc(ar, dp, True, c['s2'], c['n2'], Nn[name + '.cb2'], d_r, ACT_RELU, accumulate=False)
         if not cb2.dgrad(d_out, N, dp, accumulate=False, bstat=dsc2):
             ops.actnorm_stats(dsc2)
-        ops.actnorm_apply2(dsc1, dsc2)
+        if coef is None:
+            ops.actnorm_apply2(dsc1, dsc2)
+        else:
+            ops.actnorm_run(dsc2, stats_done=True)
         s1, raw = c['s1'], c['src_raw']
         cb1.wgrad(s1, d_r, inline)
-        short.wgrad(raw, d_sc, inline)
+        if coef is None:
+            short.wgrad(raw, d_sc, inline)
         dp1 = ar.alloc((N,) + cb1.buf_dims + (s1.C,), self.dtype)
         inp = c['inp']
         if len(inp) == 1:
@@ -521,7 +530,10 @@
             if not stats_done:
                 ops.actnorm_stats(dsc)
             a_low, a_skip = not low.first_write(), not skip.first_write()
-            if not short.dgrad_concat_norm(d_sc, N, dsc, low.C, low.grad, skip.grad, acc_low=a_low, acc_skip=a_skip):
+            if coef is not None:
+                served = short.dgrad_concat_norm(d_out, N, dsc, low.C, low.grad, skip.grad, acc_low=a_low, acc_skip=a_skip, sc=sc.data, coef=coef)
+                assert served, 'shortcut_moments serves only shapes of the split launch'
+            elif not short.dgrad_concat_norm(d_sc, N, dsc, low.C, low.grad, skip.grad, acc_low=a_low, acc_skip=a_skip):
                 dcat = ar.alloc((N,) + tuple(cb1.in_dims) + (s1.C,), self.dtype)
                 ops.actnorm_set_dx(dsc, dcat)
                 ops.actnorm_run(dsc, stats_done=True)
diff --git a/van_gan_amd/ops.py b/van_gan_amd/ops.py
--- a/van_gan_amd/ops.py
+++ b/van_gan_amd/ops.py
@@ -292,6 +292,7 @@
 FORK_SHORT = os.environ.get('VG_FORK_SHORT', '1') != '0'
 FUSE_CONCAT_NORM = os.environ.get('VG_FUSE_CONCAT_NORM', '1') != '0'
 FUSE_CONCAT = os.environ.get('VG_FUSE_CONCAT', '1') != '0'
+SHORTCUT_MOMENTS = os.environ.get('VG_SHORTCUT_MOMENTS', '1') != '0'
 BSTAT = os.environ.get('VG_BSTAT', '1') != '0'
 BSTAT_DMA = os.environ.get('VG_BSTAT_DMA', '0') != '0'
 SIDE: Optional[bool] = None
@@ -1002,22 +1003,47 @@
         D_, H_, W_ = self.in_dims
         check(lib.vg_cells_fold(_p(cells), N, D_, H_, W_, _p(dx), s_), 'vg_cells_fold ' + self.name)
 
+    def shortcut_moments(self, ar: 'Arena', src: Src, g: torch.Tensor, gamma, st: dict, dgamma, dbeta) -> Optional[torch.Tensor]:
+        if not (SHORTCUT_MOMENTS and DRY is None and not self.f32 and self.dtype == torch.bfloat16 and self.k == 1 and self.stride == 1
+                and src.x1 is not None and src.scale is None and g.dtype == torch.bfloat16
+                and FUSE_CONCAT and FUSE_CONCAT_NORM and len(self.d_classes) == 1 and not self.d_fused):
+            return None
+        d = self._fwd_desc(src)
+        s_ = stream()
+        conv_scratch(d, s_, g.device.index)
+        coef = ar.alloc((src.N, self.cout, 3), torch.float32)
+        e0 = PROF.begin() if PROF is not None else None
+        rc = lib.vg_shortcut_moments(C.byref(d), _p(g), _p(self.w), _p(gamma), _p(st['mean']), _p(st['rstd']), 1, _p(self.gw_w),
+                                     _p(dgamma), _p(dbeta), _p(coef), s_)
+        if rc < 0:
+            check(rc, 'vg_shortcut_moments ' + self.name)
+        if rc != 0:
+            return None
+        if e0 is not None:
+            PROF.end('conv_wgrad', 2.0 * src.N * math.prod(self.out_dims) * self.cout * self.cin, e0,
+                     src.N * 2 * (math.prod(self.in_dims) * self.cin + math.prod(self.out_dims) * self.cout),
+                     'shortcut_moments<%d,%d>' % (self.cin // 16, self.cout // 16), self.name)
+        return coef
+
     def dgrad_concat_norm(self, dy: torch.Tensor, N: int, nd: 'ActNormBwdDesc', c_low: int, dlow: torch.Tensor, dskip: torch.Tensor,
-                          acc_low: bool, acc_skip: bool) -> bool:
+                          acc_low: bool, acc_skip: bool, sc: Optional[torch.Tensor] = None, coef: Optional[torch.Tensor] = None) -> bool:
         if not (FUSE_CONCAT and FUSE_CONCAT_NORM and DRY is None and not self.f32 and self.k == 1 and self.stride == 1
                 and len(self.d_classes) == 1 and not self.d_fused):
             return False
         c = self.d_classes[0]
         d = self._sc_desc(dy, N)
         e0 = PROF.begin() if PROF is not None else None
-        rc = lib.vg_shortcut_dgrad_concat_norm(C.byref(d), C.byref(nd), _p(dlow), _p(dskip), c_low,
-                                               int(bool(acc_low)) | (int(bool(acc_skip)) << 1), stream())
+        acc = int(bool(acc_low)) | (int(bool(acc_skip)) << 1)
+        if coef is not None:
+            rc = lib.vg_shortcut_dgrad_concat_norm_affine(C.byref(d), C.byref(nd), _p(sc), _p(coef), _p(dlow), _p(dskip), c_low, acc, stream())
+        else:
+            rc = lib.vg_shortcut_dgrad_concat_norm(C.byref(d), C.byref(nd), _p(dlow), _p(dskip), c_low, acc, stream())
         if rc < 0:
             check(rc, 'vg_shortcut_dgrad_concat_norm ' + self.name)
         if rc == 0 and e0 is not None:
             PROF.end('conv_dgrad', 2.0 * N * math.prod(c['iters']) * self.cin * self.cout, e0,
                      N * 2 * (math.prod(self.out_dims) * self.cout + math.prod(self.buf_dims) * self.cin),
-                     'pw_gemm_split<%d,%d,n1>' % ((self.cout + 31) // 32, self.cin // 16), self.name)
+                     'pw_gemm_split<%d,%d,n1%s>' % ((self.cout + 31) // 32, self.cin // 16, '' if coef is None else ',affine'), self.name)
         return rc == 0
 
     def dgrad_concat(self, dy: torch.Tensor, N: int, dcat: torch.Tensor, c_low: int, dlow: torch.Tensor, dskip: torch.Tensor,
```

New measurement: 125.2 Mvoxels/s (median of 6 runs). About the same (+0.9%).
